# sml2004/CUDA-powered-mesh-handling-and-Iterative-solvers

Hardware: AMD Instinct MI355X
Metric: CG iterations/sec + DOFs/sec (assembly+solve), 10M P1-tet Poisson, 1/2/4/8 MI355X (higher is better)
Workload: dtype f64; 1 GPU; 10,110,954-tet P1 poisson Kuhn cube n=119, Jacobi-PCG fixed iterations; tets=10110954, nodes=1728000, dofs=1728000, nnz_blocks=25575838, parallelism=single GPU

## Files before the change

### cuda-powered-mesh-handling-and-iterative-solvers_amd/_capi.py

```python
from __future__ import annotations

import atexit
import ctypes
import functools
import inspect
import os
import threading

import torch

PKG_DIR = os.path.dirname(os.path.abspath(__file__))
LIB_PATH = os.environ.get("FEM355_LIB", os.path.join(PKG_DIR, "lib", "libfem355.so"))

FEM_OK, FEM_EBADTYPE, FEM_ESINGULAR, FEM_EHIP, FEM_ERCCL, FEM_EARG, FEM_ESTATE = range(7)
(PCG_RUNNING, PCG_CONVERGED, PCG_MAXITER, PCG_BREAKDOWN, PCG_ALPHA_NAN, PCG_BETA_NAN, PCG_SYNC_TIMEOUT,
 PCG_BAD_WINDOW) = range(8)
MODE_CG_STABLE, MODE_PCG, MODE_CG_CONSTRAINED = 0, 1, 2
TUNE_UPD1 = 1024
TUNE_U2_HOLD, TUNE_U2_SMALL = 2048, 4096
TUNE_MF_GATHER = 8192
TUNE_PK_GV = 16384
TUNE_PK_OFFDIAG = 32768
TUNE_PK_DESC = 65536
TUNE_DEFAULT = 1 | 2 | 4 | 8 | 128 | TUNE_UPD1 | TUNE_PK_OFFDIAG | TUNE_PK_DESC
KIND_ELASTIC, KIND_POISSON, KIND_MASS = 0, 1, 2
ISO_SUM, ISO_STACK, ISO_VOLUME, ISO_MASS = 0, 1, 2, 3
MASS_SELL, MASS_DIAG = 0, 1
MAT_SVK, MAT_NEO_HOOKEAN = 0, 1
MATERIALS = {"svk": MAT_SVK, "neo_hookean": MAT_NEO_HOOKEAN}
MAT_LINEAR = 2
EXPLICIT_MATERIALS = {"linear": MAT_LINEAR, **MATERIALS}
SURFACE_KINDS = {"plane": 0, "sphere": 1, "cylinder": 2}
XD_MAX_SURFACES = 8
SHELL_LOCAL, SHELL_POINTS, SHELL_GLOBAL = 0, 1, 2
LOAD_NONE, LOAD_UNIFORM, LOAD_NODAL, LOAD_ELEMENT = 0, 1, 2, 3
MODAL_OUT_GM, MODAL_OUT_NORMS, MODAL_OUT_LEN = 576, 1152, 1168

_P = ctypes.c_void_p
_I = ctypes.c_int
_L = ctypes.c_int64
_D = ctypes.c_double

SIGNATURES = {
    "fem_last_error": (ctypes.c_char_p, []),
    "fem_version": (_I, []),
    "fem_tet4_ke": (_I, [_P, _P, _L, _D, _D, _I, _P, _P, _P]),
    "fem_tet4_geom": (_I, [_P, _P, _L, _P, _P, _P, _P, _P]),
    "fem_iso_ke": (_I, [_P, _P, _L, _I, _D, _D, _P, _P, _I, _I, _P, _P]),
    "fem_iso_geom": (_I, [_P, _P, _L, _I, _P, _P, _P, _P, _P]),
    "fem_ke_sym_stride": (_I, [_I]),
    "fem_iso_ke_sym": (_I, [_P, _P, _L, _I, _D, _D, _P, _P, _I, _I, _P, _P]),
    "fem_assemble_from_ke_sym": (_I, [_P, _P, _I, _P, _P, _L, _P, _P, _P, _I, _I, _I, _P, _P]),
    "fem_assemble_from_ke_mass_sl": (_I, [_P, _P, _P, _I, _P, _P, _L, _P, _P, _P, _I, _I, _P, _P, _P]),
    "fem_iso_mass": (_I, [_P, _P, _L, _I, _D, _P, _P, _P, _I, _P, _P]),
    "fem_iso_mass_scalar": (_I, [_P, _P, _L, _I, _D, _P, _P, _P, _I, _P, _P]),
    "fem_pcg_scalars": (_I, [_P, ctypes.POINTER(_D)]),
    "fem_scan_work_len": (_L, [_L]),
    "fem_incidence_work_bytes": (_L, [_L, _L]),
    "fem_incidence": (_I, [_P, _L, _I, _L, _P, _P, _P, _P]),
    "fem_incidence_checked": (_I, [_P, _L, _I, _L, _P, _P, _P, _P, _P]),
    "fem_rcm_work_len": (_L, [_L]),
    "fem_rcm": (_I, [_P, _P, _L, _P, _P, _P, _P, _P]),
    "fem_graph_count": (_I, [_P, _I, _P, _P, _L, _P, _P, _P]),
    "fem_graph_fill": (_I, [_P, _I, _P, _P, _L, _P, _P, _P, _P]),
    "fem_graph_tmp_len": (_L, [_L]),
    "fem_graph_count2": (_I, [_P, _I, _P, _P, _L, _P, _P, _P, _P]),
    "fem_graph_fill2": (_I, [_P, _I, _P, _P, _L, _P, _P, _P, _P, _P]),
    "fem_graph_sell_fill": (_I, [_P, _I, _P, _P, _L, _P, _P, _P, _P, _P, _P, _P, _P, _P, _P]),
    "fem_graph_sell_fill_sl": (_I, [_P, _I, _P, _P, _L, _P, _P, _P, _P, _P, _P, _P, _I, _P, _P, _P, _P, _P]),
    "fem_scan_i32": (_I, [_P, _L, _P, _P, _P]),
    "fem_scan_i64": (_I, [_P, _L, _P, _P, _P]),
    "fem_sell_widths": (_I, [_P, _L, _P, _P]),
    "fem_graph_sizes": (_I, [_P, _P, _P, _L, _P, _P, _P, _P]),
    "fem_sell_fill": (_I, [_P, _P, _L, _P, _P, _P, _P]),
    "fem_sell_csr2sell": (_I, [_P, _L, _P, _P, _P]),
    "fem_assemble_from_ke": (_I, [_P, _P, _I, _I, _P, _P, _L, _P, _P, _P, _P, _P, _P]),
    "fem_assemble_from_ke_ex": (_I, [_P, _P, _I, _I, _P, _P, _L, _P, _P, _P, _P, _L, _L, _I, _P, _P]),
    "fem_assemble_from_ke_ex2": (_I, [_P, _P, _I, _I, _P, _P, _L, _P, _P, _P, _P, _L, _L, _I, _I, _P, _P]),
    "fem_assemble_tet4": (_I, [_P, _P, _D, _D, _I, _P, _P, _L, _P, _P, _P, _P, _P, _P, _P]),
    "fem_assemble_tet4_ex": (_I, [_P, _P, _D, _D, _I, _P, _P, _L, _P, _P, _P, _P, _I, _P, _P, _P]),
    "fem_assemble_tet4_ex2": (_I, [_P, _P, _D, _D, _I, _P, _P, _L, _P, _P, _P, _P, _I, _I, _P, _P, _P]),
    "fem_sell_to_csr_vals": (_I, [_P, _I, _P, _L, _P, _P, _P, _P]),
    "fem_jacobi": (_I, [_P, _I, _P, _P, _P, _P, _L, _P, _P, _P]),
    "fem_ebe_apply": (_I, [_P, _P, _I, _I, _P, _P, _L, _P, _P, _P]),
    "fem_ebe_diag": (_I, [_P, _P, _I, _I, _P, _P, _L, _I, _P, _P]),
    "fem_invert_diag": (_I, [_P, _L, _P, _P]),
    "fem_tet4_stress": (_I, [_P, _P, _L, _P, _D, _D, _P, _P, _P, _P]),
    "fem_iso_stress": (_I, [_P, _P, _L, _I, _P, _D, _D, _P, _P, _I, _I, _P, _P, _P]),
    "fem_voigt_to_tensor": (_I, [_P, _L, _P, _P]),
    "fem_von_mises": (_I, [_P, _L, _P, _P]),
    "fem_node_average": (_I, [_P, _I, _P, _P, _L, _P, _P]),
    "fem_face_forces": (_I, [_P, _P, _L, _I, _P, _P]),
    "fem_shared_face_sum": (_I, [_P, _P, _I, _L, _P, _P]),
    "fem_topo_create": (_I, [_P, _L, _I, _P, _I, _I, _L, _P, ctypes.POINTER(_P)]),
    "fem_topo_counts": (_I, [_P, ctypes.POINTER(_L), ctypes.POINTER(_L), ctypes.POINTER(_L)]),
    "fem_topo_pairs": (_I, [_P, _P]),
    "fem_topo_unique": (_I, [_P, _P]),
    "fem_topo_boundary": (_I, [_P, _P, _I, _P, _P, _P, _P, _P, ctypes.POINTER(_L)]),
    "fem_topo_destroy": (None, [_P]),
    "fem_sub_elements": (_I, [_P, _L, _I, _P, _I, _I, _P, _P]),
    "fem_element_face_normals": (_I, [_P, _P, _L, _I, _P, _P, _P, _P, _I, _D, _I, _I, _P, _P]),
    "fem_surface_normals": (_I, [_P, _P, _P, _L, _I, _I, _P, _P]),
    "fem_solid_ke": (_I, [_I, _P, _P, _L, _D, _D, _P, _P, _I, _I, _P, _P]),
    "fem_csr_pattern": (_I, [_P, _L, _I, _I, _L, _P, _P, _P, ctypes.POINTER(_L), _P]),
    "fem_csr_fill": (_I, [_P, _P, _L, _I, _I, _L, _P, _P, _P, _P]),
    "fem_spmv_csr": (_I, [_P, _P, _P, _P, _P, _L, _P]),
    "fem_pcg_csr": (_I, [_P, _P, _P, _L, _P, _P, _P, _P, _D, _I, _D, _I, ctypes.POINTER(_I), ctypes.POINTER(_I), _P,
                         _P]),
    "fem_vtk_read": (_I, [ctypes.c_char_p, ctypes.POINTER(_P)]),
    "fem_vtk_sizes": (_I, [_P, ctypes.POINTER(_L), ctypes.POINTER(_L), ctypes.POINTER(_L), ctypes.POINTER(_L)]),
    "fem_vtk_copy": (_I, [_P, _P, _P, _P]),
    "fem_vtk_free": (None, [_P]),
    "fem_spmv": (_I, [_L, _I, _P, _P, _P, _P, _P, _P]),
    "fem_sell_delta16": (_I, [_P, _L, _P, _P, _P, _P]),
    "fem_spmv16": (_I, [_L, _I, _P, _P, _P, _P, _P, _P]),
    "fem_pcg_set_cols16": (_I, [_P, _P]),
    "fem_pcg_set_tuning": (_I, [_P, _I]),
    "fem_stream_copy": (_I, [_P, _P, _L, _I, _P]),
    "fem_stream_read": (_I, [_P, _P, _L, _I, _P]),
    "fem_pcg_create": (_I, [_L, _I, _P, _P, _P, _P, _P, _P, _I, _D, _D, _P, _L, _P, ctypes.POINTER(_P)]),
    "fem_pcg_start": (_I, [_P]),
    "fem_pcg_iterate": (_I, [_P, _I]),
    "fem_pcg_poll": (_I, [_P, ctypes.POINTER(_I), ctypes.POINTER(_I), ctypes.POINTER(_D)]),
    "fem_pcg_sync_site": (_I, [_P, ctypes.POINTER(_I)]),
    "fem_pcg_debug_window": (_I, [_P, _I, _I, _I]),
    "fem_pcg_solve": (_I, [_P, _I, _I, ctypes.POINTER(_I), ctypes.POINTER(_I), ctypes.POINTER(_D)]),
    "fem_pcg_use_graph": (_I, [_P, _I]),
    "fem_pcg_set_schedule": (_I, [_P, _I]),
    "fem_pcg_set_entries": (_I, [_P, _L]),
    "fem_pcg_get_schedule": (_I, [_P]),
    "fem_pcg_uniform_slices": (_I, [_P, _L, _L, _P, _P, _P]),
    "fem_pcg_offdiag_slices": (_I, [_P, _P, _P, _P]),
    "fem_pcg_debug_offdiag": (_I, [_P, _P, _P]),
    "fem_pcg_desc_slices": (_I, [_P, _P, _P]),
    "fem_pcg_debug_desc": (_I, [_P, _P]),
    "fem_pcg_persist_build": (_I, [_P, ctypes.POINTER(_I), ctypes.POINTER(_I), ctypes.POINTER(_I)]),
    "fem_pcg_pipelined": (_I, [_P, ctypes.POINTER(_I)]),
    "fem_sell_sl_pattern": (_I, [_L, _P, _P, _I, _P, _P, _P, _P, _P]),
    "fem_assemble_tet4_sl": (_I, [_P, _P, _D, _D, _I, _P, _P, _L, _P, _P, _P, _P, _P, _I, _I, _P, _P, _P]),
    "fem_assemble_from_ke_sl": (_I, [_P, _P, _I, _P, _P, _L, _P, _P, _P, _I, _I, _P, _P]),
    "fem_jacobi_sl": (_I, [_P, _I, _P, _P, _P, _P, _P, _L, _P, _P, _P]),
    "fem_spmv_sl": (_I, [_L, _I, _P, _P, _P, _P, _P, _P, _P, _P]),
    "fem_sell_sl_unpair": (_I, [_L, _I, _P, _P, _P, _P, _P, _P, _P, _P]),
    "fem_pcg_set_layout": (_I, [_P, _P, _P, _P, _P, _P, _I]),
    "fem_pcg_persist_profile": (_I, [_P, _I, _P, ctypes.POINTER(_I)]),
    "fem_pcg_set_constraints": (_I, [_P, _I, _L, _P, _P, _L, _P, _P, _L, _P, _P, _P, _P, _P]),
    "fem_enforce_constraints": (_I, [_P, _P, _L, _I, _L, _P, _P, _L, _P, _P, _L, _P, _P, _P, _P, _P, _P]),
    "fem_pcg_finish": (_I, [_P]),
    "fem_pcg_profile": (_I, [_P, _I, _I, ctypes.POINTER(_D), ctypes.POINTER(_I)]),
    "fem_pcg_destroy": (None, [_P]),
    "fem_pcg_release_cache": (_I, []),
    "fem_release_scratch": (_I, []),
    "fem_pcg_set_rows": (_I, [_P, _I, _I, _P, _I]),
    "fem_pcg_comm_block": (_I, [_P, ctypes.POINTER(_P), ctypes.POINTER(_L)]),
    "fem_pcg_col_window": (_I, [_P, ctypes.POINTER(_L), ctypes.POINTER(_L)]),
    "fem_pcg_set_peers": (_I, [_P, _P, _P, _P]),
    "fem_pcg_dist_debug": (_I, [_P, _I, _P, _L]),
    "fem_stream_create_cu": (_I, [_I, _I, ctypes.POINTER(_P)]),
    "fem_stream_destroy": (_I, [_P]),
    "fem_pcg_set_prof": (_I, [_P, _P]),
    "fem_ipc_handle": (_I, [_P, ctypes.c_char_p]),
    "fem_ipc_open": (_I, [ctypes.c_char_p, ctypes.POINTER(_P)]),
    "fem_ipc_close": (_I, [_P]),
    "fem_sell_diag": (_I, [_P, _I, _P, _P, _L, _P, _P]),
    "fem_jacobi_from_diag": (_I, [_P, _L, _P, _P, _P]),
    "fem_mf_create": (_I, [_P, _P, _L, _L, _I, _D, _D, ctypes.POINTER(_L), _P, ctypes.POINTER(_P)]),
    "fem_mf_destroy": (_I, [_P]),
    "fem_mf_apply": (_I, [_P, _P, _P, _P]),
    "fem_mf_diag": (_I, [_P, _P, _P]),
    "fem_mf_info": (_I, [_P, ctypes.POINTER(_L)]),
    "fem_mf_order": (_I, [_P, _P, _P, _P, _P, _P]),
    "fem_pcg_set_operator_mf": (_I, [_P, _P]),
    "fem_comm_unique_id": (_I, [ctypes.c_char_p]),
    "fem_comm_init": (_I, [_I, _I, ctypes.c_char_p, ctypes.POINTER(_P)]),
    "fem_comm_destroy": (_I, [_P]),
    "fem_allreduce_sum": (_I, [_P, _P, _L, _P]),
    "fem_halo_sum": (_I, [_P, _P, _I, _P, _L, _P, _L, _P, _P]),
    "fem_halo_pack": (_I, [_P, _I, _P, _L, _P, _P]),
    "fem_halo_unpack": (_I, [_P, _I, _P, _L, _P, _P]),
    "fem_pcg_set_dist": (_I, [_P, _I, _P, _L, _P, _P, _P]),
    "fem_pcg_set_dist_variant": (_I, [_P, _I]),
    "fem_pcg_set_p2p": (_I, [_P, _I, _I, _P, _P, _P, _P]),
    "fem_pcg_p2p_buffers": (_I, [_P, ctypes.POINTER(_P), ctypes.POINTER(_P), ctypes.POINTER(_L)]),
    "fem_p2p_deliver": (_I, [_P, _I, _P]),
    "fem_pcg_dist_phase": (_I, [_P, _I]),
    "fem_pcg_dist_buffer": (_I, [_P, _I, ctypes.POINTER(_P), ctypes.POINTER(_L)]),
    "fem_group_allreduce": (_I, [_P, _I, _L, _P]),
    "fem_spmm": (_I, [_L, _I, _I, _P, _P, _P, _P, _P, _P, _P]),
    "fem_mpcg_create": (_I, [_L, _I, _I, _I, _P, _P, _P, _P, _P, _P, _P, _I, ctypes.POINTER(_D), _D, _P, _L, _P,
                             ctypes.POINTER(_P)]),
    "fem_mpcg_solve": (_I, [_P, _I, _I, ctypes.POINTER(_I), ctypes.POINTER(_I), ctypes.POINTER(_D)]),
    "fem_mpcg_scalars": (_I, [_P, ctypes.POINTER(_D)]),
    "fem_mpcg_destroy": (None, [_P]),
    "fem_coarse_restrict": (_I, [_L, _I, _I, _P, _P, _P, _P, _P, _P, _P]),
    "fem_coarse_apply": (_I, [_L, _I, _I, _P, _P, _P, _P, _P, _P, _P, _P, _P]),
    "fem_coarse_galerkin_count": (_I, [_L, _I, _P, _P, _P, _P, _P, _P]),
    "fem_coarse_galerkin": (_I, [_L, _I, _I, _P, _P, _P, _P, _P, _P, _P, _P, _P, _P, _P]),
    "fem_coarse_galerkin_sum": (_I, [_L, _I, _P, _P, _P, _P, _P, _P]),
    "fem_pcg2_create": (_I, [_L, _I, _P, _P, _P, _P, _P, _P, _P, _I, _P, _P, _P, _P, _P, _D, _P, _L, _P,
                             ctypes.POINTER(_P)]),
    "fem_pcg2_solve": (_I, [_P, _I, _I, ctypes.POINTER(_I), ctypes.POINTER(_I), ctypes.POINTER(_D)]),
    "fem_pcg2_scalars": (_I, [_P, ctypes.POINTER(_D)]),
    "fem_pcg2_destroy": (None, [_P]),
    "fem_refine_edge_slots": (_I, [_P, _L, _P, _L, _P, _P, _P]),
    "fem_refine_emit": (_I, [_P, _L, _L, _P, _P, _P, _P]),
    "fem_refine_nodes": (_I, [_P, _L, _P, _L, _P, _P, _P, _P]),
    "fem_mg_restrict": (_I, [_L, _L, _I, _P, _P, _P, _P, _P, _P]),
    "fem_mg_prolong": (_I, [_L, _L, _I, _P, _P, _P, _P, _P]),
    "fem_mg_create": (_I, [_I, _I, _P, _P, _P, _P, _P, _P, _P, _P, _P, _I, _P, _P, _L, _P, _P, ctypes.POINTER(_P)]),
    "fem_mg_apply": (_I, [_P, _P, _P]),
    "fem_mg_sweep": (_I, [_P, _I]),
    "fem_mg_solve": (_I, [_P, _P, _P, _D, _I, _I, _P, _L, ctypes.POINTER(_I), ctypes.POINTER(_I),
                          ctypes.POINTER(_D)]),
    "fem_mg_scalars": (_I, [_P, ctypes.POINTER(_D)]),
    "fem_mg_destroy": (None, [_P]),
    "fem_spmm_km": (_I, [_L, _I, _I, _P, _P, _P, _P, _P, _I, _P, _P, _P, _P]),
    "fem_modal_work_len": (_L, []),
    "fem_modal_gram": (_I, [_L, _I, _I, ctypes.POINTER(_P), _P, _P, _P]),
    "fem_modal_residual": (_I, [_L, _I, _P, _P, _P, _P, _P, _P, _P, _P]),
# ... 165 lines not shown
```

### cuda-powered-mesh-handling-and-iterative-solvers_amd/csrc/pcg.hip

```cpp
#include <rccl/rccl.h>
#include <stddef.h>

#include <atomic>
#include <mutex>
#include <vector>

#include "sell_pair.hpp"
#include "sell_pair3.hpp"
#include "matfree.hpp"

namespace fem {

template <typename T, bool NT>
__device__ __forceinline__ T ld(const T* p) {
    if constexpr (NT) return __builtin_nontemporal_load(p);
    else return *p;
}

struct VecPlain {
    const double* x;
    __device__ __forceinline__ double operator()(int64_t i) const { return x[i]; }
};
struct VecFusedP {
    const double* r;
// ... 1630 lines not shown
    for (int64_t i = (int64_t)blockIdx.x * blockDim.x + threadIdx.x; i < n; i += (int64_t)gridDim.x * blockDim.x)
        if (w[i] == 0.0) x[i] = 0.0;
}

}

using namespace fem;

struct fem_pcg {
    int64_t nrows, nslices, n;
    int bs;
    const int64_t* slice_ptr;
    const int32_t* cols;
    const double* vals;
    const double* b;
    double* x;
    const double* w;
    double* hist;
    int64_t hist_len;
    int mode;
    double tol, eps;
    hipStream_t stream;
    int fused;
    int deferred;
    int64_t launched;
    int64_t sell_ent;
    const int16_t* cols16;
    int has_con;
    int tune;
    int paired;
    double* pvals;
    int16_t* pcols16;
    int32_t* puoff;
    int16_t* pucol;
    int pext;
    const int32_t* pwin_ext;
    int pwin_G;
    Constraints con;
    double* r;
    double* p0;
    double* p1;
    double* q;
    RedBuf red;
    PcgState* st;
    PcgState* st_host;
    int grid_spmv, grid_vec;
    hipGraphExec_t graph;
    int graph_k;
    int max_iter;
    int dist;
    ncclComm_t comm;
    int64_t nI;
    const int32_t* imap;
    const int32_t* ipos;
    const uint8_t* own;
    double* hbuf;
    int cg1;
    double* cg1_s;
    double* cg1_u;
    double* cg1_send;
    double* cg1_recv;
    int p2p;
    int p2p_nranks;
    std::vector<int> peer_rank;
    std::vector<int64_t> peer_off, peer_cnt;
    int64_t p2p_total;
    const int32_t* p2p_csrc;
    const int32_t* p2p_ssrc;
    double* psend;
    double* precv;
    int c1f;
    int c1f_grid;
    int c1f_win_ok;
    int32_t* c1f_win;
    unsigned* c1f_flags;
    int persist_req;
    int persist_fit_only;
    int persist;
    int pk_grid;
    int pk_win_ok;
    int32_t* pk_win;
    double* pk_part;
    unsigned* pk_sync;
    int pk_ovf;
    double* pk_v;
    int pk_od;
    double* pk_ovals;
    int16_t* pk_oucol;
    int32_t* pk_kd;
    double* pk_diag;
    PkDesc* pk_desc;
    int pk_desc_on;
    int pk_coop;
    int pk_gv;
    double* gv_buf;
    int64_t gv_cap;
    int gv_init_pending;
    int64_t pk_epochs;
    hipEvent_t pev[2];
    int pd;
    int pd_rank, pd_nranks, pd_grid_req;
    int64_t pd_split[PK_MAX_RANKS + 1];
    char* pd_block;
    int64_t pd_block_bytes, pd_off_flag, pd_off_red, pd_off_rflag;
    int64_t pd_off_m1;
    char* pd_peer[PK_MAX_RANKS];
    int pd_peers_ok;
    int32_t* pd_pub;
    int pd_init_pending;
    unsigned long long* pd_prof;
    int upd1;
    int u2_grid;
    unsigned* u2_sync;
    fem_mf* mf;
    double* mf_sl;
    int64_t mf_sl_cap;
    int mf_nogather;
    int mf_qfuse;
};

#define FEM_NCCL(call)                                                                         \
    do {                                                                                       \
        ncclResult_t _r = (call);                                                              \
        if (_r != ncclSuccess) {                                                               \
            ::fem::set_error("%s:%d %s -> %s", __FILE__, __LINE__, #call, ncclGetErrorString(_r)); \
            return FEM_ERCCL;                                                                  \
        }                                                                                      \
    } while (0)

static const int16_t* pcols(const fem_pcg* s) { return s->bs == 1 ? s->pcols16 : s->cols16; }

template <class CI>
struct col_type {
    using type = CI;
};

template <class F>
static auto with_bs(int bs, F&& f) {
    return bs == 3 ? f(std::integral_constant<int, 3>{}) : f(std::integral_constant<int, 1>{});
}

template <class F>
static auto with_matrix(const fem_pcg* s, bool paired, F&& f) {
    return with_bs(s->bs, [&](auto B) {
        if (paired) return f(B, col_type<int16_t>{}, std::true_type{}, pcols(s), (const double*)s->pvals);
        if (s->cols16) return f(B, col_type<int16_t>{}, std::false_type{}, s->cols16, s->vals);
        return f(B, col_type<int32_t>{}, std::false_type{}, s->cols, s->vals);
    });
}
template <class F>
static auto with_matrix(const fem_pcg* s, F&& f) {
    return with_matrix(s, s->paired != 0, f);
}

static double* st_red(fem_pcg* s, int k) {
    return reinterpret_cast<double*>(reinterpret_cast<char*>(s->st) + offsetof(PcgState, red)) + k;
}

template <int BS>
__global__ void __launch_bounds__(MF_BLOCK) k_pcg_mf_dot(MfOp op, const double* __restrict__ p,
                                                         double* __restrict__ slots, PcgState* __restrict__ st,
                                                         RedBuf red) {
    __shared__ MfLds<BS> L;
    __shared__ double lds4[MF_BLOCK / 64];
    __shared__ int flag;
    if (blockIdx.x == 0 && threadIdx.x == 0) st->xupd = 0;
// ... 685 lines not shown
static const int64_t CON_SMALL = 8192;
static int launch_constraints(hipStream_t stream, double* x, double* r, const Constraints& c, const PcgState* st,
                              int always) {
    if (c.R + c.S <= CON_SMALL) {
        hipLaunchKernelGGL(k_constraints, dim3(1), dim3(256), 0, stream, x, r, c, st, always, 3);
        FEM_LAUNCHED();
        return FEM_OK;
    }
    auto phase = [&](int ph) {
        const int64_t m = ph == CON_SPC ? c.S : c.R;
        if (m == 0) return;
        const dim3 g(stream_grid(m, 256));
        if (ph == CON_GATHER) hipLaunchKernelGGL(k_con_phase<CON_GATHER>, g, dim3(256), 0, stream, x, r, c, st, always);
        if (ph == CON_SCATTER) hipLaunchKernelGGL(k_con_phase<CON_SCATTER>, g, dim3(256), 0, stream, x, r, c, st, always);
        if (ph == CON_SPC) hipLaunchKernelGGL(k_con_phase<CON_SPC>, g, dim3(256), 0, stream, x, r, c, st, always);
    };
    if (c.order == 0) {
        phase(CON_GATHER);
        phase(CON_SCATTER);
        phase(CON_SPC);
    } else {
        phase(CON_SPC);
        phase(CON_GATHER);
        phase(CON_SCATTER);
        if (c.G) hipLaunchKernelGGL(k_constraints, dim3(1), dim3(256), 0, stream, x, r, c, st, always, 2);
    }
    FEM_LAUNCHED();
    return FEM_OK;
}

static int launch_pupdate(fem_pcg* s) {
    if (s->fused) return FEM_OK;
    hipLaunchKernelGGL(k_pcg_pupdate, dim3(s->grid_vec), dim3(PCG_BLOCK), 0, s->stream, s->n, s->x, s->p0, s->r, s->w,
                       s->st);
    FEM_LAUNCHED();
    if (s->has_con) return launch_constraints(s->stream, s->x, nullptr, s->con, s->st, 0);
    return FEM_OK;
}

static int launch_update_finish(fem_pcg* s) {
    int rc;
    if ((rc = launch_update(s))) return rc;
    if (!s->dist) return FEM_OK;
    if ((rc = dist_exchange(s, 2))) return rc;
    hipLaunchKernelGGL(k_fin_rz, dim3(1), dim3(1), 0, s->stream, s->st, s->hist, s->hist_len);
    FEM_LAUNCHED();
    return FEM_OK;
}

static int launch_deferred(fem_pcg* s, int which) {
    const int par = (int)(s->launched & 1);
    const int rev = (s->tune & FEM_TUNE_REVERSE) ? par : 0;
    if (which == 0) {
        with_matrix(s, [&](auto B, auto ci, auto PAIR, auto* cols, const double* vals) {
            hipLaunchKernelGGL((k_pcg_d1<B(), typename decltype(ci)::type, PAIR()>), dim3(s->grid_spmv),
                               dim3(PCG_BLOCK), 0, s->stream, s->nslices, s->nrows, s->slice_ptr, cols, vals, s->p0, s->q,
                               s->st, par, rev, s->red.partials);
        });
    } else if (which == 1) {
        hipLaunchKernelGGL(k_pcg_d2, dim3(s->grid_vec), dim3(PCG_BLOCK), 0, s->stream, s->n, s->r, s->q, s->w, s->st,
                           par, s->red.partials, s->grid_spmv, s->red.partials + MAX_PARTIALS);
    } else {
        hipLaunchKernelGGL(k_pcg_d3, dim3(s->grid_vec), dim3(PCG_BLOCK), 0, s->stream, s->n, s->x, s->p0, s->r, s->w,
                           s->st, par, s->red.partials + MAX_PARTIALS, s->grid_vec, s->hist, s->hist_len);
        s->launched++;
    }
    FEM_LAUNCHED();
    return FEM_OK;
}

enum PkFamily { PKF_BS1, PKF_BS1_DIST, PKF_BS3, PKF_GV };

struct PkBuild {
    PkFamily fam;
    int slots;
    bool prof;
    bool gsc1;
    bool ovf;
    bool dist;
    bool od;
    const void* fn;
    size_t lds;
    bool desc;
};

template <int MAXS, bool PROF, bool GSC1, bool OVF = false, bool DIST = false, bool OD = false, bool DESC = false>
static PkBuild pk1_build() {
    return {DIST ? PKF_BS1_DIST : PKF_BS1, MAXS, PROF, GSC1, OVF, DIST, OD,
            (const void*)k_pcg_persist<MAXS, PROF, GSC1, OVF, DIST, OD, DESC>, PK_LDS, DESC};
}
template <bool OVF, bool DIST>
static PkBuild pk3_build() {
    return {PKF_BS3, P3_MAXS, false, true, OVF, DIST, false, (const void*)k_pcg_persist3<P3_MAXS, OVF, DIST>, P3_LDS};
}
template <int MAXS, bool DIST>
static PkBuild gv_build() {
    return {PKF_GV, MAXS, false, true, false, DIST, false, (const void*)k_pcg_persist_gv<MAXS, DIST>, GV_LDS};
}

constexpr int PK_MAXS_DIST = 4;

static const PkBuild PK_BUILDS[] = {
    pk1_build<1, false, true>(),
    pk1_build<2, false, true>(),
    pk1_build<4, false, true>(),
    pk1_build<PK_MAXS, false, true>(),
    pk1_build<PK_MAXS, false, false>(),
    pk1_build<PK_MAXS, true, true>(),
    pk1_build<PK_MAXS, true, false>(),
    pk1_build<PK_MAXS, false, true, true>(),
    pk1_build<PK_MAXS, false, false, true>(),
    pk1_build<1, false, true, false, false, true>(),
    pk1_build<2, false, true, false, false, true>(),
    pk1_build<4, false, true, false, false, true>(),
    pk1_build<PK_MAXS, false, true, false, false, true>(),
    pk1_build<PK_MAXS, false, false, false, false, true>(),
    pk1_build<PK_MAXS, true, true, false, false, true>(),
    pk1_build<PK_MAXS, true, false, false, false, true>(),
    pk1_build<PK_MAXS, false, true, true, false, true>(),
    pk1_build<PK_MAXS, false, false, true, false, true>(),
    pk1_build<1, false, true, false, false, true, true>(),
    pk1_build<2, false, true, false, false, true, true>(),
    pk1_build<4, false, true, false, false, true, true>(),
    pk1_build<PK_MAXS, false, true, false, false, true, true>(),
    pk1_build<PK_MAXS, true, true, false, false, true, true>(),
    pk1_build<1, false, true, false, true>(),
    pk1_build<2, false, true, false, true>(),
    pk1_build<PK_MAXS_DIST, false, true, false, true>(),
    pk1_build<PK_MAXS_DIST, true, true, false, true>(),
    pk1_build<PK_MAXS, false, true, false, true>(),
    pk1_build<PK_MAXS, true, true, false, true>(),
    pk3_build<false, false>(),
    pk3_build<true, false>(),
    pk3_build<false, true>(),
    gv_build<1, false>(),
    gv_build<2, false>(),
    gv_build<1, true>(),
    gv_build<2, true>(),
};

static const PkBuild* pk_find(PkFamily fam, int slots, bool prof, bool gsc1, bool ovf, bool dist, bool od,
                              bool desc = false) {
    for (const PkBuild& b : PK_BUILDS)
        if (b.fam == fam && b.slots == slots && b.prof == prof && b.gsc1 == gsc1 && b.ovf == ovf && b.dist == dist &&
            b.od == od && b.desc == desc)
            return &b;
    return nullptr;
}

static int pk_max_slots(PkFamily fam) {
    int m = 0;
    for (const PkBuild& b : PK_BUILDS)
        if (b.fam == fam && b.slots > m) m = b.slots;
    return m;
}

static int pk_pack(int64_t nslices, int G) {
    const int64_t maxL = (nslices + G - 1) / G;
    return (int)((maxL + PK_WAVES - 1) / PK_WAVES);
}

static int64_t pk_own_slices(const fem_pcg* s) {
    return s->pd ? s->pd_split[s->pd_rank + 1] - s->pd_split[s->pd_rank] : s->nslices;
}

struct PkPlan {
    const PkBuild* b;
    int pack;
};

static PkPlan persist_plan(const fem_pcg* s, bool prof, bool gv) {
    const int pk = pk_pack(pk_own_slices(s), s->pk_grid);
    const bool dist = s->pd != 0;
    if (gv) return {pk_find(PKF_GV, pk <= 1 ? 1 : 2, false, true, false, dist, false), pk};
    if (s->bs == 3) return {pk_find(PKF_BS3, P3_MAXS, false, true, !dist && s->pk_ovf, dist, false), pk};
    if (dist) {
        const int slots = !prof && pk <= 1 ? 1 : !prof && pk == 2 ? 2 : pk <= PK_MAXS_DIST ? PK_MAXS_DIST : PK_MAXS;
        return {pk_find(PKF_BS1_DIST, slots, prof, true, false, true, false), pk};
    }
    const int pack = (s->tune & FEM_TUNE_PK_PACK) ? pk : 0;
    const bool ovf = s->pk_ovf != 0, gsc1 = (s->tune & FEM_TUNE_PK_SC1) != 0;
    prof = prof && !ovf;
    const bool small = pack >= 1 && pack <= 4 && !(s->tune & FEM_TUNE_PK_WIDE) && !prof && !ovf && gsc1;
    const int slots = !small ? PK_MAXS : pack == 1 ? 1 : pack == 2 ? 2 : 4;
    const bool desc = s->pk_od && s->pk_desc_on && gsc1 && !ovf;
    return {pk_find(PKF_BS1, slots, prof, gsc1, ovf, false, s->pk_od != 0, desc), pack};
}
static PkPlan persist_plan(const fem_pcg* s, bool prof) { return persist_plan(s, prof, s->pk_gv && s->bs == 1); }

static int check_resident(const void* fn, int threads, size_t lds, int* nb) {
    FEM_HIP(hipFuncSetAttribute(fn, hipFuncAttributeMaxDynamicSharedMemorySize, (int)lds));
    FEM_HIP(hipOccupancyMaxActiveBlocksPerMultiprocessor(nb, fn, threads, lds));
    return FEM_OK;
}

static int family_resident(PkFamily fam, bool dist, int* res) {
    *res = 1;
    for (const PkBuild& b : PK_BUILDS) {
        if (b.fam != fam || b.dist != dist) continue;
        int nb = 0;
        const int rc = check_resident(b.fn, PK_T, b.lds, &nb);
        if (rc) return rc;
        if (nb < 1) {
            *res = 2;
            break;
        }
    }
    return FEM_OK;
}

static int launch_persist(fem_pcg* s, int k, unsigned long long* prof = nullptr);

static int launch_iterations(fem_pcg* s, int k) {
    if (s->dist && !s->comm) {
        set_error("distributed PCG without a communicator: drive it with fem_pcg_dist_phase");
        return FEM_EARG;
    }
    if (s->persist) return launch_persist(s, k);
    if (s->deferred && !s->dist) {
        for (int i = 0; i < k; ++i) {
            int rc;
            if ((rc = launch_deferred(s, 0)) || (rc = launch_deferred(s, 1)) || (rc = launch_deferred(s, 2))) return rc;
        }
        return FEM_OK;
    }
    if (s->dist && s->cg1) {
        for (int i = 0; i < k; ++i) {
            int rc;
            if ((rc = dist_phase(s, 4)) || (rc = dist_exchange(s, 4))) return rc;
            s->launched++;
        }
        return FEM_OK;
    }
    for (int i = 0; i < k; ++i) {
        int rc;
        if ((rc = launch_spmv_dot(s))) return rc;
        if (s->upd1) {
            if ((rc = launch_update2(s))) return rc;
        } else {
            if ((rc = launch_exchange_dot(s))) return rc;
            if ((rc = launch_update_finish(s))) return rc;
            if ((rc = launch_pupdate(s))) return rc;
        }
        s->launched++;
    }
    return FEM_OK;
}

template <class CI>
static int spmv_plain(const char* fn, int64_t nrows, int bs, const int64_t* slice_ptr, const CI* cols,
                      const double* vals, const double* x, double* y, fem_stream_t stream) {
    const int64_t ns = cdiv(nrows, 64);
    if (ns == 0) return FEM_OK;
    if (bs != 1 && bs != 3) {
        set_error("%s: block size %d unsupported", fn, bs);
        return FEM_EARG;
    }
    const int grid = grid_multiple_of_xcd(cdiv(ns, 4), 2048);
    with_bs(bs, [&](auto B) {
        hipLaunchKernelGGL((k_spmv<B(), SPMV_U, false, CI>), dim3(grid), dim3(256), 0, S(stream), ns, nrows, slice_ptr,
                           cols, vals, x, y);
    });
    FEM_LAUNCHED();
    return FEM_OK;
}

extern "C" {

// ... 76 lines not shown
    }
    Constraints c;
    const int rc = make_constraints("fem_pcg_set_constraints", s->n, s->stream, order, R, rbe2_slave, rbe2_master, S,
                                    spc_dof, spc_val, G, r3_ptr, r3_master, r3_wsum, r3_slave, r3_w, &c);
    if (rc != FEM_OK) return rc;
    if (s->con.tmp) (void)hipFree(s->con.tmp);
    s->con.tmp = nullptr;
    if (R > 0) FEM_HIP(hipMalloc(&c.tmp, sizeof(double) * (size_t)R));
    s->con = c;
    s->has_con = 1;
    return FEM_OK;
}

int fem_enforce_constraints(double* x, double* r, int64_t n, int order, int64_t R, const int64_t* rbe2_slave,
                            const int64_t* rbe2_master, int64_t S, const int64_t* spc_dof, const double* spc_val,
                            int64_t G, const int64_t* r3_ptr, const int64_t* r3_master, const double* r3_wsum,
                            const int64_t* r3_slave, const double* r3_w, fem_stream_t stream) {
    if (!x || n < 0) {
        set_error("fem_enforce_constraints: null x / negative n");
        return FEM_EARG;
    }
    const hipStream_t st = reinterpret_cast<hipStream_t>(stream);
    Constraints c;
    const int rc = make_constraints("fem_enforce_constraints", n, st, order, R, rbe2_slave, rbe2_master, S, spc_dof,
                                    spc_val, G, r3_ptr, r3_master, r3_wsum, r3_slave, r3_w, &c);
    if (rc != FEM_OK) return rc;
    if (R > 0) FEM_HIP(::fem::malloc_async((void**)&c.tmp, sizeof(double) * (size_t)R, st));
    const int lrc = launch_constraints(st, x, r, c, nullptr, 1);
    if (lrc != FEM_OK) return lrc;
    if (c.tmp) FEM_HIP(hipFreeAsync(c.tmp, st));
    return FEM_OK;
}

int fem_pcg_set_tuning(fem_pcg* s, int flags) {
    if (s->graph) {
        set_error("fem_pcg_set_tuning: drop the captured graph first");
        return FEM_EARG;
    }
    s->tune = flags;
    return FEM_OK;
}

int fem_pcg_set_cols16(fem_pcg* s, const int16_t* dcols) {
    if (s->graph) {
        set_error("fem_pcg_set_cols16: drop the captured graph first");
        return FEM_EARG;
    }
    s->cols16 = dcols;
    if (!dcols) s->paired = 0;
    return FEM_OK;
}

int fem_stream_copy(const double* src, double* dst, int64_t n, int grid, fem_stream_t stream) {
    if (grid <= 0) grid = 2048;
    hipLaunchKernelGGL(k_stream_copy, dim3(grid), dim3(256), 0, S(stream), (const double2*)src, (double2*)dst, n / 2);
    FEM_LAUNCHED();
    return FEM_OK;
}

int fem_stream_read(const double* src, double* out, int64_t n, int grid, fem_stream_t stream) {
    if (grid <= 0) grid = 4096;
    hipLaunchKernelGGL(k_stream_read, dim3(grid), dim3(256), 0, S(stream), (const double2*)src, n / 2, out);
    FEM_LAUNCHED();
    return FEM_OK;
}

int fem_pcg_create(int64_t nrows, int bs, const int64_t* slice_ptr, const int32_t* cols, const double* vals,
                   const double* b, double* x, const double* w, int mode, double tol, double eps, double* hist,
                   int64_t hist_len, fem_stream_t stream, fem_pcg** out) {
    if (bs != 1 && bs != 3) {
        set_error("fem_pcg_create: block size %d unsupported", bs);
        return FEM_EARG;
    }
    if (mode != FEM_MODE_CG_STABLE && mode != FEM_MODE_PCG && mode != FEM_MODE_CG_CONSTRAINED) {
        set_error("fem_pcg_create: unknown mode %d", mode);
        return FEM_EARG;
    }
    if (((uintptr_t)b | (uintptr_t)x | (uintptr_t)w) & 15) {
        set_error("fem_pcg_create: vectors must be 16-byte aligned");
        return FEM_EARG;
    }
    fem_pcg* s = new fem_pcg();
    s->tune = FEM_TUNE_REVERSE | FEM_TUNE_PAIR | FEM_TUNE_PK_SC1 | FEM_TUNE_PK_PACK | FEM_TUNE_PK_UNI | FEM_TUNE_UPD1 |
              FEM_TUNE_PK_OFFDIAG | FEM_TUNE_PK_DESC;
    s->nrows = nrows;
    s->bs = bs;
    s->nslices = cdiv(nrows, 64);
    s->n = nrows * bs;
    s->sell_ent = -1;
    s->slice_ptr = slice_ptr;
    s->cols = cols;
    s->vals = vals;
    s->b = b;
    s->x = x;
    s->w = w;
    s->hist = hist;
    s->hist_len = hist ? hist_len : 0;
    s->mode = mode;
    s->tol = tol;
    s->eps = eps;
    s->stream = S(stream);
    s->fused = 0;
    s->graph = nullptr;
    s->graph_k = 0;
    s->max_iter = 0x7fffffff;
    s->grid_spmv = grid_multiple_of_xcd(cdiv(s->nslices, 4), 2048);
    s->grid_vec = grid_multiple_of_xcd(cdiv(s->n / 2 + 1, PCG_BLOCK), 1024);
    size_t vec = sizeof(double) * (size_t)(s->n + 2);
    hipError_t e = hipSuccess;
    if (e == hipSuccess) e = pool_alloc((void**)&s->r, vec, s->stream, s->bs == 1);
    if (e == hipSuccess) e = pool_alloc((void**)&s->p0, vec, s->stream, s->bs == 1);
    if (e == hipSuccess) e = pool_alloc((void**)&s->p1, vec, s->stream, s->bs == 1);
    if (e == hipSuccess) e = pool_alloc((void**)&s->q, vec, s->stream, s->bs == 1);
    if (e == hipSuccess)
        e = pool_alloc((void**)&s->red.partials, sizeof(double) * RED_N * MAX_PARTIALS, s->stream, s->bs == 1);
    if (e == hipSuccess)
        e = pool_alloc((void**)&s->red.counters, sizeof(unsigned) * RED_N * RED_COUNTER_WORDS, s->stream, s->bs == 1);
    if (e == hipSuccess) e = hipMemsetAsync(s->red.counters, 0, sizeof(unsigned) * RED_N * RED_COUNTER_WORDS, s->stream);
    if (e == hipSuccess) e = pool_alloc((void**)&s->st, sizeof(PcgState), s->stream, s->bs == 1);
    if (e == hipSuccess) e = host_state_alloc((void**)&s->st_host, sizeof(PcgState));
    if (e != hipSuccess) {
        set_error("fem_pcg_create: allocation failed: %s", hipGetErrorString(e));
        fem_pcg_destroy(s);
        return FEM_EHIP;
    }
    *out = s;
    return FEM_OK;
}

int fem_pcg_set_operator_mf(fem_pcg* s, fem_mf* m) {
    if (!s || !m || mf_bs(m) != s->bs || mf_nodes(m) != s->nrows) {
        set_error("fem_pcg_set_operator_mf: the operator's block size / node count do not match the context");
        return FEM_EARG;
    }
    if (s->pd || s->has_con || s->graph || s->mode == FEM_MODE_CG_CONSTRAINED) {
        set_error("fem_pcg_set_operator_mf: contexts without constraints (CG_STABLE / PCG mode), the row-partitioned "
                  "schedule or a captured graph only");
        return FEM_EARG;
    }
    if (s->dist && !s->cg1) {
        set_error("fem_pcg_set_operator_mf: a distributed context runs the element-chunk operator in the "
                  "single-reduction variant only (fem_pcg_set_dist_variant(s, 1))");
        return FEM_EARG;
    }
    const int64_t need = (int64_t)mf_bs(m) * (int64_t)mf_nslots(m);
    if (need > s->mf_sl_cap) {
        if (s->mf_sl) FEM_HIP(hipFree(s->mf_sl));
        s->mf_sl = nullptr;
        s->mf_sl_cap = 0;
        FEM_HIP(hipMalloc(&s->mf_sl, sizeof(double) * (size_t)need));
        s->mf_sl_cap = need;
    }
    s->mf = m;
    {
        const char* e = getenv("FEM355_MF_NOGATHER");
        s->mf_nogather = e ? (atoi(e) != 0) : (int)(mf_nodes(m) >= MF_NOGATHER_MIN_NODES);
    }
    s->fused = s->deferred = s->persist_req = s->persist_fit_only = s->persist = 0;
    s->cols16 = nullptr;
    s->pext = 0;
    return FEM_OK;
}

int fem_pcg_set_entries(fem_pcg* s, int64_t entries) {
    if (entries < 0) {
        set_error("fem_pcg_set_entries: negative entry count %lld", (long long)entries);
        return FEM_EARG;
// ... 243 lines not shown
        for (int32_t k : h) c += k >= 0;
    }
    *od_slices = c;
    *bytes = c * 64 * (int64_t)sizeof(double);
    return FEM_OK;
}

static bool pk_runs_desc(const fem_pcg* s) {
    if (!s->persist || !s->pk_od || s->bs != 1 || s->pd || s->pk_gv) return false;
    const PkBuild* b = persist_plan(s, false, false).b;
    return b && b->desc;
}

int fem_pcg_desc_slices(fem_pcg* s, int64_t* desc_slices, int64_t* nslices) {
    *desc_slices = 0;
    *nslices = s->nslices;
    if (!pk_runs_desc(s) || s->nslices == 0) return FEM_OK;
    std::vector<PkDesc> h((size_t)s->nslices);
    FEM_HIP(hipMemcpyAsync(h.data(), s->pk_desc, sizeof(PkDesc) * h.size(), hipMemcpyDeviceToHost, s->stream));
    FEM_HIP(hipStreamSynchronize(s->stream));
    int64_t c = 0;
    for (const PkDesc& d : h) c += ((d.w[3] >> 8) & 0xffu) != (uint32_t)PKD_LANE;
    *desc_slices = c;
    return FEM_OK;
}

int fem_pcg_debug_desc(fem_pcg* s, uint32_t* records) {
    if (!pk_runs_desc(s)) {
        set_error("fem_pcg_debug_desc: the started context reads no descriptor records");
        return FEM_EARG;
    }
    FEM_HIP(hipMemcpyAsync(records, s->pk_desc, sizeof(PkDesc) * (size_t)s->nslices, hipMemcpyDeviceToHost, s->stream));
    FEM_HIP(hipStreamSynchronize(s->stream));
    return FEM_OK;
}

int fem_pcg_debug_offdiag(fem_pcg* s, const int32_t* rowptr, double* vals) {
    if (!s->persist || !s->pk_od || !s->cols16) {
        set_error("fem_pcg_debug_offdiag: the started context reads no diagonal-free stream");
        return FEM_EARG;
    }
    hipLaunchKernelGGL(k_sell_od_unpair, dim3(stream_grid(s->nslices * 64, 256)), dim3(256), 0, s->stream, s->nslices,
                       s->slice_ptr, s->cols16, s->puoff, s->pucol, s->pk_kd, s->pk_diag, rowptr, s->nrows,
                       s->pk_ovals, vals);
    FEM_LAUNCHED();
    FEM_HIP(hipStreamSynchronize(s->stream));
    return FEM_OK;
}

static int persist_setup(fem_pcg* s) {
    s->persist = 0;
    s->pk_od = 0;
    if (s->pd) return persist_setup_dist(s);
    if (!s->persist_req) return FEM_OK;
    if ((s->bs != 1 && s->bs != 3) || !s->paired || s->dist || s->mode == FEM_MODE_CG_CONSTRAINED || s->nslices == 0)
        return FEM_OK;
    int dev = 0, ncu = 0;
    FEM_HIP(hipGetDevice(&dev));
    FEM_HIP(hipDeviceGetAttribute(&ncu, hipDeviceAttributeMultiprocessorCount, dev));
    const int G = (ncu / NXCD) * NXCD;
    if (G < NXCD) return FEM_OK;
    const PkFamily fam = s->bs == 3 ? PKF_BS3 : PKF_BS1;
    const bool ovf = s->nslices > (int64_t)G * PK_WAVES * pk_max_slots(fam);
    if (ovf && (!(s->tune & FEM_TUNE_PK_PACK) || s->persist_fit_only)) return FEM_OK;
    static std::mutex occ_mu;
    static int occ_cache[2][64] = {};
    int occ;
    {
        std::lock_guard<std::mutex> lk(occ_mu);
        int& slot = occ_cache[s->bs == 3][dev & 63];
        if (slot == 0) {
            int res = 0;
            const int rc = family_resident(fam, false, &res);
            if (rc) return rc;
            slot = res;
        }
        occ = slot;
    }
    if (occ != 1) return FEM_OK;
    if (s->pk_grid != G) {
        pool_free(s->pk_win, s->stream);
        pool_free(s->pk_part, s->stream);
        pool_free(s->pk_sync, s->stream);
        s->pk_win = nullptr;
        s->pk_part = nullptr;
        s->pk_sync = nullptr;
        FEM_HIP(pool_alloc((void**)&s->pk_win, sizeof(int32_t) * 2 * G, s->stream, s->bs == 1));
        FEM_HIP(pool_alloc((void**)&s->pk_part, sizeof(double) * 4 * G, s->stream, s->bs == 1));
        FEM_HIP(pool_alloc((void**)&s->pk_sync, sizeof(unsigned) * pk_sync_words(G), s->stream, s->bs == 1));
        s->pk_grid = G;
        s->pk_win_ok = 0;
    }
    if (!s->pk_win_ok && s->pwin_ext && s->pwin_G == G) {
        FEM_HIP(hipMemcpyAsync(s->pk_win, s->pwin_ext, sizeof(int32_t) * 2 * G, hipMemcpyDeviceToDevice, s->stream));
        s->pk_win_ok = 1;
    }
    if (!s->pk_win_ok) {
        hipLaunchKernelGGL(k_pk_window_init, dim3(cdiv(G, 256)), dim3(256), 0, s->stream, G, G, s->pk_win);
        FEM_LAUNCHED();
        hipLaunchKernelGGL(k_pk_window, dim3(stream_grid(s->nslices * 64, 256)), dim3(256), 0, s->stream, s->nslices,
                           s->nrows, s->slice_ptr, s->cols16, G, s->pk_win, s->pk_win + G);
        FEM_LAUNCHED();
        s->pk_win_ok = 1;
    }
    if (ovf && !s->pk_v) FEM_HIP(pool_alloc((void**)&s->pk_v, sizeof(double) * (size_t)s->n, s->stream, s->bs == 1));
    s->pk_ovf = ovf ? 1 : 0;
    s->persist = 1;
    s->pk_gv = 0;
    if ((s->tune & FEM_TUNE_PK_GV) && (s->tune & FEM_TUNE_PK_SC1) && s->bs == 1 && !ovf && s->mode == FEM_MODE_PCG) {
        if (pk_pack(s->nslices, G) <= pk_max_slots(PKF_GV)) {
            static std::mutex gv_mu;
            static int gv_ok[64] = {};
            std::lock_guard<std::mutex> lk(gv_mu);
            int& slot = gv_ok[dev & 63];
            if (slot == 0) {
                int res = 0;
                const int rc = family_resident(PKF_GV, false, &res);
                if (rc) return rc;
                slot = res;
            }
            s->pk_gv = slot == 1;
        }
    }
    return offdiag_build(s);
}

static int persist_setup_dist(fem_pcg* s) {
    if ((s->bs != 1 && s->bs != 3) || !s->paired || s->dist || s->mode == FEM_MODE_CG_CONSTRAINED) {
        set_error("distributed persistent PCG: needs bs = 1 or 3, 16-bit columns with the paired copy, no element "
                  "partition, no constraints");
        return FEM_EARG;
    }
    if (!s->pd_peers_ok) {
        set_error("distributed persistent PCG: fem_pcg_set_peers first");
        return FEM_EARG;
    }
    const int G = s->pk_grid;
    const int64_t nloc = pk_own_slices(s);
    if ((nloc + G - 1) / G > (int64_t)PK_WAVES * pk_max_slots(s->bs == 3 ? PKF_BS3 : PKF_BS1_DIST)) {
        set_error("distributed persistent PCG: %lld slices on this rank exceed the register capacity of %d workgroups",
                  (long long)nloc, G);
        return FEM_EARG;
    }
    s->pk_ovf = 0;
    s->pk_gv = 0;
    for (int prof = 0; prof < (s->bs == 3 ? 1 : 2); ++prof) {
        const PkBuild* b = persist_plan(s, prof != 0, false).b;
        int nb = 0;
        const int rc = b ? check_resident(b->fn, PK_T, b->lds, &nb) : FEM_OK;
        if (rc) return rc;
        if (nb < 1) {
            set_error("distributed persistent PCG: kernel does not fit one workgroup per CU");
            return FEM_EARG;
        }
    }
    s->persist = 1;
    if (s->pd_off_m1 > 0 && s->mode == FEM_MODE_PCG && pk_pack(nloc, G) <= pk_max_slots(PKF_GV)) {
        int res = 0;
        const int rc = family_resident(PKF_GV, true, &res);
        if (rc) return rc;
        s->pk_gv = res == 1;
    }
    return FEM_OK;
}

static int persist_reset_sync(fem_pcg* s) {
    FEM_HIP(hipMemsetAsync(s->pk_sync, 0, sizeof(unsigned) * pk_sync_words(s->pk_grid), s->stream));
    FEM_HIP(hipMemsetAsync(&s->st->pk_epoch, 0, sizeof(unsigned), s->stream));
    s->pk_epochs = 0;
    return FEM_OK;
}

static PkArgs pk_args(const fem_pcg* s, const PkPlan& plan, int k, unsigned long long* prof) {
    const bool bs3 = s->bs == 3;
    const bool uni = (s->tune & FEM_TUNE_PK_UNI) && s->puoff;
    const bool od = plan.b->od;
    PkArgs a;
    a.nslices = pk_own_slices(s);
    a.nrows = s->nrows;
    a.slice_ptr = s->slice_ptr;
    a.cols = pcols(s);
    a.vals = od ? s->pk_ovals : s->pvals;
    a.uoff = uni && !bs3 ? s->puoff : nullptr;
    a.ucol = bs3 ? nullptr : od ? s->pk_oucol : uni ? s->pucol : nullptr;
    a.x = s->x;
    a.r = s->r;
    a.p = s->p0;
    a.s = s->p1;
    a.u = s->pd ? reinterpret_cast<double*>(s->pd_block) : s->q;
    a.w = s->w;
    a.win = s->pk_win;
    a.part = s->pk_part;
    a.sync = s->pk_sync;
    a.st = s->st;
    a.hist = s->hist;
    a.hist_len = s->hist_len;
    a.kmax = k;
    a.rev = (s->tune & FEM_TUNE_REVERSE) ? 1 : 0;
    a.prof = prof;
    a.v = s->pk_ovf ? s->pk_v : nullptr;
    a.pack = plan.pack;
    a.sbase = s->pd ? s->pd_split[s->pd_rank] : 0;
    a.rank = s->pd ? s->pd_rank : 0;
    a.nranks = s->pd ? s->pd_nranks : 1;
    for (int q = 0; q < PK_MAX_RANKS; ++q) a.peer[q] = s->pd && q < s->pd_nranks ? s->pd_peer[q] : nullptr;
    a.off_flag = s->pd ? s->pd_off_flag : 0;
    a.off_red = s->pd ? s->pd_off_red : 0;
    a.off_rflag = s->pd ? s->pd_off_rflag : 0;
    a.pub = s->pd ? s->pd_pub : nullptr;
    a.b = s->b;
    a.init = s->pd ? s->pd_init_pending : 0;
    a.diag = od ? s->pk_diag : nullptr;
    a.vals_full = s->pvals;
    a.ucol_full = uni ? s->pucol : nullptr;
    a.desc = plan.b->desc ? s->pk_desc : nullptr;
    return a;
}

static GvArgs gv_args(const fem_pcg* s) {
    const int64_t n = s->n;
    GvArgs g;
    g.u = s->gv_buf;
    g.w = s->gv_buf + n;
    g.q = s->gv_buf + 2 * n;
    g.z = s->gv_buf + 3 * n;
    g.m[0] = s->pd ? reinterpret_cast<double*>(s->pd_block) : s->gv_buf + 4 * n;
    g.m[1] = s->pd ? reinterpret_cast<double*>(s->pd_block + s->pd_off_m1) : s->gv_buf + 5 * n;
    g.moff[0] = 0;
    g.moff[1] = s->pd ? s->pd_off_m1 : 0;
    g.init = s->pd ? 0 : s->gv_init_pending;
    return g;
}

static int launch_persist(fem_pcg* s, int k, unsigned long long* prof) {
    const int G = s->pk_grid;
    if (s->pk_epochs + k + 1 > (int64_t(1) << 24)) {
        if (s->pd) {
            set_error("distributed persistent PCG: 2^24 iterations since fem_pcg_start; restart the solve");
            return FEM_EARG;
        }
        const int rc = persist_reset_sync(s);
        if (rc) return rc;
    }
    s->pk_epochs += k + 1;
    const bool gv = s->pk_gv && s->bs == 1;
    if (prof && (gv || (s->bs == 3 && !s->pd))) {
        set_error("persistent PCG: no instrumented (PROF) build %s", gv ? "of the pipelined iteration" : "for bs = 3");
        return FEM_EARG;
    }
    if (s->pd && !prof && !gv) prof = s->pd_prof;
    if (s->bs == 3) prof = nullptr;
    const PkPlan plan = persist_plan(s, prof != nullptr);
    if (!plan.b) {
        set_error("persistent PCG: no build for this context (%d slices per wave)", plan.pack);
        return FEM_ESTATE;
    }
    PkArgs a = pk_args(s, plan, k, prof);
    s->pd_init_pending = 0;
    GvArgs g;
    void* args[] = {&a, &g};
    if (gv) {
        g = gv_args(s);
        s->gv_init_pending = 0;
        s->pk_epochs += 2;
    }
    if (s->pk_coop || (s->tune & FEM_TUNE_PK_COOP))
        FEM_HIP(hipLaunchCooperativeKernel(plan.b->fn, dim3(G), dim3(PK_T), args, plan.b->lds, s->stream));
    else
        FEM_HIP(hipLaunchKernel(plan.b->fn, dim3(G), dim3(PK_T), args, plan.b->lds, s->stream));
    FEM_LAUNCHED();
    s->launched += k;
    return FEM_OK;
}

int fem_pcg_pipelined(fem_pcg* s, int* on) {
    *on = (s && s->persist && s->pk_gv) ? 1 : 0;
    return FEM_OK;
}

int fem_pcg_persist_build(fem_pcg* s, int* slots, int* overflow, int* pack) {
    *slots = 0;
    *overflow = 0;
    *pack = 0;
    if (!s->persist || s->pk_grid <= 0) return FEM_OK;
    const PkPlan plan = persist_plan(s, false, false);
    *slots = plan.b ? plan.b->slots : 0;
    *overflow = s->pk_ovf;
    *pack = plan.pack;
    return FEM_OK;
}

__global__ void __launch_bounds__(256) k_sell_sl_pattern(int64_t nslices, int64_t nrows,
                                                         const int64_t* __restrict__ slice_ptr,
                                                         const int16_t* __restrict__ cin, int16_t* __restrict__ pout,
                                                         int16_t* __restrict__ ucol, int32_t* __restrict__ uoff, int G,
                                                         int* __restrict__ win, int2* __restrict__ span) {
    __shared__ int cand_all[4][SU_MAXW];
    const int64_t s = ((int64_t)blockIdx.x * blockDim.x + threadIdx.x) >> 6;
    if (s >= nslices) return;
    const int l = threadIdx.x & 63;
    const int64_t p0 = slice_ptr[s];
    sl_pattern_slice(s, l, nslices, nrows, slice_ptr, [&](int k) { return (int)cin[p0 + 64 * k + l]; }, pout, ucol,
                     uoff, G, win, cand_all[(threadIdx.x >> 6) & 3], span);
}

static PcgState state_view(const fem_pcg* s) {
    PcgState h = *s->st_host;
    if (s->deferred && !s->dist && !s->persist) {
        const PcgState::Bank& b = h.bank[s->launched & 1];
        h.iter = b.iter;
        h.status = b.status;
        h.halt = b.halt;
        h.stop_iter = b.stop_iter;
        h.rz = b.rz;
        h.rz_new = b.rz_new;
        h.pq = b.pq;
        h.alpha = b.alpha;
        h.beta = b.beta;
    }
    return h;
}

static int refresh_pairing(fem_pcg* s) {
    const bool want = (s->bs == 1 || s->bs == 3) && s->cols16 && (s->tune & FEM_TUNE_PAIR) && !s->fused;
    s->paired = 0;
    if (s->pext) {
        if (!want) {
            set_error("PCG: a solver-layout matrix needs the paired schedules (FEM_TUNE_PAIR, 16-bit columns, not fused)");
            return FEM_EARG;
        }
        s->paired = 1;
        return FEM_OK;
    }
    if (!want || s->nslices == 0) return FEM_OK;
    int64_t ent = s->sell_ent;
    if (ent < 0) {
        FEM_HIP(hipMemcpyAsync(&ent, s->slice_ptr + s->nslices, sizeof(int64_t), hipMemcpyDeviceToHost, s->stream));
        FEM_HIP(hipStreamSynchronize(s->stream));
    }
    if (s->bs == 3) {
        if (!s->pvals) FEM_HIP(pool_alloc((void**)&s->pvals, sizeof(double) * 9 * (size_t)ent, s->stream, s->bs == 1));
        s->pcols16 = nullptr;
        hipLaunchKernelGGL(k_sell3_to_a, dim3(stream_grid(s->nslices * 64, 256)), dim3(256), 0, s->stream, s->nslices,
                           s->slice_ptr, s->vals, s->pvals);
        FEM_LAUNCHED();
        s->paired = 1;
        return FEM_OK;
    }
    if (!s->pvals) {
        FEM_HIP(pool_alloc((void**)&s->pvals, sizeof(double) * (size_t)ent, s->stream, s->bs == 1));
        FEM_HIP(pool_alloc((void**)&s->pcols16, sizeof(int16_t) * (size_t)ent, s->stream, s->bs == 1));
    }
    s->paired = 1;
    if ((s->tune & FEM_TUNE_PK_UNI) && 2 * (ent / 64) + 2 < (int64_t)INT32_MAX) {
        if (!s->puoff) {
            FEM_HIP(pool_alloc((void**)&s->puoff, sizeof(int32_t) * (size_t)s->nslices, s->stream, true));
            FEM_HIP(pool_alloc((void**)&s->pucol, sizeof(int16_t) * (size_t)(2 * (ent / 64) + 2), s->stream, true));
        }
        hipLaunchKernelGGL(k_sell_uniform, dim3((unsigned)cdiv(s->nslices, 4)), dim3(256), 0, s->stream, s->nslices,
                           s->nrows, s->slice_ptr, s->vals, s->cols16, s->pvals, s->pcols16, s->pucol, s->puoff, 1);
        FEM_LAUNCHED();
        return FEM_OK;
    }
    hipLaunchKernelGGL(k_sell_pair, dim3(stream_grid(s->nslices * 64, 256)), dim3(256), 0, s->stream, s->nslices,
                       s->slice_ptr, s->vals, s->cols16, s->pvals, s->pcols16);
    FEM_LAUNCHED();
    return FEM_OK;
}

static int gv_ensure(fem_pcg* s) {
    const int64_t need = 6 * s->n;
    if (need > s->gv_cap) {
        pool_free(s->gv_buf, s->stream);
        s->gv_buf = nullptr;
        s->gv_cap = 0;
        FEM_HIP(pool_alloc((void**)&s->gv_buf, sizeof(double) * (size_t)need, s->stream, true));
        s->gv_cap = need;
    }
    FEM_HIP(hipMemsetAsync(s->gv_buf, 0, sizeof(double) * (size_t)need, s->stream));
    return FEM_OK;
}

int fem_pcg_start(fem_pcg* s) {
    if (s->mf && s->dist && !s->cg1) {
        set_error("fem_pcg_start: a distributed element-chunk context needs the single-reduction variant "
                  "(fem_pcg_set_dist_variant(s, 1))");
        return FEM_EARG;
    }
    {
        int prc = refresh_pairing(s);
        if (!prc) prc = persist_setup(s);
        if (!prc) prc = c1f_setup(s);
        if (!prc) prc = u2_setup(s);
        if (prc) return prc;
    }
    PcgState h{};
    h.tol = s->tol;
    h.eps = s->eps;
    h.mode = s->mode;
    h.max_iter = s->max_iter;
    h.x_done = 1;
    h.dist = s->dist;
    *s->st_host = h;
    FEM_HIP(hipMemcpyAsync(s->st, s->st_host, sizeof(PcgState), hipMemcpyHostToDevice, s->stream));
    int rc;
    if (s->dist) {
        if (!s->comm) return FEM_OK;
        if (s->cg1) {
            if ((rc = dist_phase(s, 10)) || (rc = dist_exchange(s, 10)) || (rc = dist_phase(s, 20)) ||
                (rc = dist_exchange(s, 20)))
                return rc;
            return FEM_OK;
        }
        if ((rc = dist_phase(s, 10)) || (rc = dist_exchange(s, 10)) || (rc = dist_phase(s, 11)) ||
            (rc = dist_exchange(s, 11)) || (rc = dist_phase(s, 12)))
            return rc;
        return FEM_OK;
    }
    if (s->mode == FEM_MODE_CG_STABLE) {
        hipLaunchKernelGGL(k_zero_fixed, dim3(stream_grid(s->n, 256)), dim3(256), 0, s->stream, s->n, s->x, s->w);
        FEM_LAUNCHED();
    }
    if (s->pd) {
        if (!s->persist) {
            set_error("distributed persistent PCG: setup failed");
            return FEM_EARG;
        }
        FEM_HIP(hipMemsetAsync(s->pk_sync, 0, sizeof(unsigned) * pk_sync_words(s->pk_grid), s->stream));
        FEM_HIP(hipMemsetAsync(s->pd_block, 0, (size_t)s->pd_block_bytes, s->stream));
        FEM_HIP(hipMemsetAsync(&s->st->pk_epoch, 0, sizeof(unsigned), s->stream));
        s->pk_epochs = 0;
        s->pd_init_pending = 1;
        s->launched = 0;
        if (s->pk_gv && (rc = gv_ensure(s))) return rc;
        return FEM_OK;
    }
    if ((rc = start_spmv(s, true))) return rc;
    if (s->persist) {
        const int zrc = persist_reset_sync(s);
        if (zrc) return zrc;
        if (s->pk_gv) {
            if ((rc = gv_ensure(s))) return rc;
            s->gv_init_pending = 1;
        }
        hipLaunchKernelGGL(k_cg1_init, dim3(s->grid_vec), dim3(PCG_BLOCK), 0, s->stream, s->n, s->bs, s->b, s->r,
                           s->q, s->w, s->p0, s->p1, s->q, (const uint8_t*)nullptr, s->st, s->red);
        FEM_LAUNCHED();
        s->launched = 0;
        return FEM_OK;
    }
    hipLaunchKernelGGL(k_pcg_init, dim3(s->grid_vec), dim3(PCG_BLOCK), 0, s->stream, s->n, s->b, s->r, s->q, s->w, s->p0,
                       s->p1, s->fused, s->st, s->red, (const uint8_t*)nullptr, s->bs);
    FEM_LAUNCHED();
    if (s->has_con) {
        const int rc = launch_constraints(s->stream, s->x, nullptr, s->con, s->st, 1);
        if (rc != FEM_OK) return rc;
    }
    s->launched = 0;
    if (s->deferred) {
        hipLaunchKernelGGL(k_bank_init, dim3(1), dim3(1), 0, s->stream, s->st);
        FEM_LAUNCHED();
    }
    return FEM_OK;
}

int fem_pcg_dist_phase(fem_pcg* s, int phase) {
    if (!s->dist) {
        set_error("fem_pcg_dist_phase: context is not in distributed mode");
        return FEM_EARG;
    }
    return dist_phase(s, phase);
}

int fem_pcg_dist_buffer(fem_pcg* s, int phase, double** ptr, int64_t* n) {
    dist_buffer(s, phase, ptr, n);
    return FEM_OK;
}

int fem_comm_unique_id(char* out128) {
    ncclUniqueId id;
    FEM_NCCL(ncclGetUniqueId(&id));
    memcpy(out128, id.internal, sizeof(id.internal));
    return FEM_OK;
}

int fem_comm_init(int nranks, int rank, const char* id128, void** comm) {
    ncclUniqueId id;
    memcpy(id.internal, id128, sizeof(id.internal));
    ncclComm_t c;
    FEM_NCCL(ncclCommInitRank(&c, nranks, id, rank));
    *comm = c;
    return FEM_OK;
}

int fem_comm_destroy(void* comm) {
    if (comm) FEM_NCCL(ncclCommDestroy((ncclComm_t)comm));
    return FEM_OK;
}

int fem_allreduce_sum(void* comm, double* buf, int64_t n, fem_stream_t stream) {
    FEM_NCCL(ncclAllReduce(buf, buf, (size_t)n, ncclFloat64, ncclSum, (ncclComm_t)comm, S(stream)));
    return FEM_OK;
}

int fem_halo_pack(const double* v, int bs, const int32_t* imap, int64_t nI, double* buf, fem_stream_t stream) {
    if (nI <= 0) return FEM_OK;
    hipLaunchKernelGGL(k_halo_pack, dim3(stream_grid(nI * bs, 256)), dim3(256), 0, S(stream), v, bs, imap, nI, buf,
                       (const PcgState*)nullptr, 0);
    FEM_LAUNCHED();
    return FEM_OK;
}
// ... 355 lines not shown
        const bool dfr = s->deferred && !s->dist;
        if (s->upd1) {
            (void)hipEventRecord(evs[4 * si + 0], s->stream);
            rc = launch_spmv_dot(s);
            (void)hipEventRecord(evs[4 * si + 1], s->stream);
            if (!rc) rc = launch_update2(s);
            (void)hipEventRecord(evs[4 * si + 2], s->stream);
            (void)hipEventRecord(evs[4 * si + 3], s->stream);
            s->launched++;
            ++si;
            continue;
        }
        (void)hipEventRecord(evs[4 * si + 0], s->stream);
        rc = dfr ? launch_deferred(s, 0) : launch_spmv_dot(s);
        (void)hipEventRecord(evs[4 * si + 1], s->stream);
        if (!rc && !dfr) rc = launch_exchange_dot(s);
        if (!rc) rc = dfr ? launch_deferred(s, 1) : launch_update_finish(s);
        (void)hipEventRecord(evs[4 * si + 2], s->stream);
        if (!rc) rc = dfr ? launch_deferred(s, 2) : launch_pupdate(s);
        (void)hipEventRecord(evs[4 * si + 3], s->stream);
        ++si;
    }
    FEM_HIP(hipStreamSynchronize(s->stream));
    for (int i = 0; i < si; ++i) {
        float t;
        for (int j = 0; j < 3; ++j) {
            const bool c1 = s->dist && s->cg1;
            (void)hipEventElapsedTime(&t, evs[4 * i + (c1 && j == 2 ? 3 : j)], evs[4 * i + (c1 && j == 2 ? 0 : j + 1)]);
            acc[j] += t;
        }
    }
    for (auto& e : evs) (void)hipEventDestroy(e);
    for (int j = 0; j < 3; ++j) {
        if (ms) ms[j] = acc[j];
        if (n) n[j] = si;
    }
    return rc;
}

int fem_pcg_set_rows(fem_pcg* s, int nranks, int rank, const int64_t* slice_split, int grid) {
    if (nranks < 1 || nranks > PK_MAX_RANKS || rank < 0 || rank >= nranks || !slice_split) {
        set_error("fem_pcg_set_rows: nranks %d (1..%d), rank %d", nranks, PK_MAX_RANKS, rank);
        return FEM_EARG;
    }
    if ((s->bs != 1 && s->bs != 3) || s->dist || s->mode == FEM_MODE_CG_CONSTRAINED || s->pd) {
        set_error("fem_pcg_set_rows: bs = 1 or 3, not element-partitioned, not constrained, once per context");
        return FEM_EARG;
    }
    if (slice_split[0] != 0 || slice_split[nranks] != s->nslices) {
        set_error("fem_pcg_set_rows: the split must cover slices [0, %lld)", (long long)s->nslices);
        return FEM_EARG;
    }
    for (int q = 0; q < nranks; ++q)
        if (slice_split[q + 1] <= slice_split[q]) {
            set_error("fem_pcg_set_rows: rank %d owns no slice", q);
            return FEM_EARG;
        }
    int dev = 0, ncu = 0;
    FEM_HIP(hipGetDevice(&dev));
    FEM_HIP(hipDeviceGetAttribute(&ncu, hipDeviceAttributeMultiprocessorCount, dev));
    const int G = grid > 0 ? grid : (ncu / NXCD) * NXCD;
    if (G < NXCD || G % NXCD || G > ncu) {
        set_error("fem_pcg_set_rows: grid %d must be a multiple of %d within %d CUs", G, NXCD, ncu);
        return FEM_EARG;
    }
    s->pd_rank = rank;
    s->pd_nranks = nranks;
    for (int q = 0; q <= nranks; ++q) s->pd_split[q] = slice_split[q];
    const int64_t line = sizeof(unsigned) * PK_LINE;
    const int64_t vreg = (int64_t)cdiv(sizeof(double) * (s->n + 2), 256) * 256;
    s->pd_off_m1 = ((s->tune & FEM_TUNE_PK_GV) && s->bs == 1) ? vreg : 0;
    s->pd_off_flag = vreg + s->pd_off_m1;
    s->pd_off_red = s->pd_off_flag + (int64_t)nranks * G * line;
    s->pd_off_rflag = s->pd_off_red + 256;
    s->pd_block_bytes = s->pd_off_rflag + PK_MAX_RANKS * NXCD * line;
    if (s->tune & FEM_TUNE_DIST_FINE)
        FEM_HIP(hipExtMallocWithFlags((void**)&s->pd_block, (size_t)s->pd_block_bytes, hipDeviceMallocFinegrained));
    else
        FEM_HIP(hipMalloc((void**)&s->pd_block, (size_t)s->pd_block_bytes));
    FEM_HIP(hipMemsetAsync(s->pd_block, 0, (size_t)s->pd_block_bytes, s->stream));
    pool_free(s->pk_win, s->stream);
    pool_free(s->pk_part, s->stream);
    pool_free(s->pk_sync, s->stream);
    FEM_HIP(pool_alloc((void**)&s->pk_win, sizeof(int32_t) * (2 * G + 2), s->stream, true));
    FEM_HIP(pool_alloc((void**)&s->pk_part, sizeof(double) * 4 * G, s->stream, true));
    FEM_HIP(pool_alloc((void**)&s->pk_sync, sizeof(unsigned) * pk_sync_words(G), s->stream, true));
    s->pk_grid = G;
    std::vector<int32_t> lohi(2 * (size_t)G + 2);
    for (int i = 0; i < G; ++i) {
        lohi[i] = nranks * G;
        lohi[G + i] = -1;
    }
    lohi[2 * G] = 0x7fffffff;
    lohi[2 * G + 1] = -1;
    FEM_HIP(hipMemcpyAsync(s->pk_win, lohi.data(), sizeof(int32_t) * lohi.size(), hipMemcpyHostToDevice, s->stream));
    PkSplit sp{};
    for (int q = 0; q <= nranks; ++q) sp.b[q] = slice_split[q];
    const int64_t nloc = slice_split[rank + 1] - slice_split[rank];
    hipLaunchKernelGGL(k_pk_window_dist, dim3(stream_grid(nloc * 64, 256)), dim3(256), 0, s->stream, slice_split[rank],
                       nloc, s->nrows, s->slice_ptr, s->cols, G, sp, nranks, s->pk_win, s->pk_win + G,
                       s->pk_win + 2 * G);
    FEM_LAUNCHED();
    FEM_HIP(hipStreamSynchronize(s->stream));
    s->pk_win_ok = 1;
    s->pd = 1;
    s->pd_peers_ok = 0;
    s->persist_req = 1;
    s->deferred = 1;
    s->fused = 0;
    return FEM_OK;
}

int fem_pcg_comm_block(fem_pcg* s, void** base, int64_t* bytes) {
    if (!s->pd) {
        set_error("fem_pcg_comm_block: fem_pcg_set_rows first");
        return FEM_EARG;
    }
    if (base) *base = s->pd_block;
    if (bytes) *bytes = s->pd_block_bytes;
    return FEM_OK;
}

int fem_pcg_col_window(fem_pcg* s, int64_t* lo, int64_t* hi) {
    if (!s->pd) {
        set_error("fem_pcg_col_window: fem_pcg_set_rows first");
        return FEM_EARG;
    }
    int32_t w[2];
    FEM_HIP(hipMemcpyAsync(w, s->pk_win + 2 * s->pk_grid, sizeof w, hipMemcpyDeviceToHost, s->stream));
    FEM_HIP(hipStreamSynchronize(s->stream));
    *lo = w[0];
    *hi = w[1];
    return FEM_OK;
}

int fem_pcg_set_peers(fem_pcg* s, void* const* bases, const int64_t* need_lo, const int64_t* need_hi) {
    if (!s->pd) {
        set_error("fem_pcg_set_peers: fem_pcg_set_rows first");
        return FEM_EARG;
    }
    const int N = s->pd_nranks, G = s->pk_grid, r = s->pd_rank;
    for (int q = 0; q < N; ++q) {
        s->pd_peer[q] = q == r ? s->pd_block : (char*)bases[q];
        if (!s->pd_peer[q]) {
            set_error("fem_pcg_set_peers: no comm block for rank %d", q);
            return FEM_EARG;
        }
    }
    const int64_t S0 = s->pd_split[r], nloc = s->pd_split[r + 1] - S0;
    auto owner = [&](int64_t row) {
        const int64_t sl = row >> 6;
        int q = 0;
        while (q + 1 < N && s->pd_split[q + 1] <= sl) ++q;
        const int64_t S = s->pd_split[q + 1] - s->pd_split[q], tl = sl - s->pd_split[q];
        const int64_t L = ((tl + 1) * G - 1) / S;
        return (int64_t)q * G + (L < G ? L : G - 1);
    };
    std::vector<int32_t> pub((size_t)G * N * 2, -1);
    for (int q = 0; q < N && !(s->tune & FEM_TUNE_DIST_DROP); ++q) {
        if (q == r || need_hi[q] < need_lo[q]) continue;
        const int64_t glo = owner(need_lo[q]), ghi = owner(need_hi[q]);
        for (int L = 0; L < G; ++L) {
            const int64_t Lg = (int64_t)r * G + L;
            if (Lg < glo || Lg > ghi) continue;
            const int64_t rlo = (S0 + (int64_t)L * nloc / G) * 64;
            const int64_t rhi = std::min<int64_t>((S0 + (int64_t)(L + 1) * nloc / G) * 64, s->nrows);
            const int64_t lo = std::max<int64_t>(rlo, need_lo[q]), hi = std::min<int64_t>(rhi, need_hi[q] + 1);
            pub[((size_t)L * N + q) * 2] = (int32_t)std::max<int64_t>(lo, 0);
            pub[((size_t)L * N + q) * 2 + 1] = (int32_t)std::max<int64_t>(hi, std::max<int64_t>(lo, 0));
// ... 44 lines not shown
        return FEM_EARG;
    }
    std::vector<uint32_t> mask((size_t)(ncu + 31) / 32, 0u);
    for (int cu = 0; cu < ncu; ++cu)
        if (cu % nparts == part) mask[(size_t)cu / 32] |= 1u << (cu % 32);
    hipStream_t st = nullptr;
    FEM_HIP(hipExtStreamCreateWithCUMask(&st, (uint32_t)mask.size(), mask.data()));
    *stream = st;
    return FEM_OK;
}

int fem_stream_destroy(void* stream) {
    FEM_HIP(hipStreamDestroy(reinterpret_cast<hipStream_t>(stream)));
    return FEM_OK;
}

int fem_pcg_set_prof(fem_pcg* s, unsigned long long* dev_buf) {
    if (!s->pd) {
        set_error("fem_pcg_set_prof: distributed persistent contexts only (single GPU: fem_pcg_persist_profile)");
        return FEM_EARG;
    }
    s->pd_prof = dev_buf;
    return FEM_OK;
}

int fem_ipc_handle(void* ptr, char* out64) {
    hipIpcMemHandle_t h;
    FEM_HIP(hipIpcGetMemHandle(&h, ptr));
    static_assert(sizeof(h) <= 64, "IPC handle size");
    memset(out64, 0, 64);
    memcpy(out64, &h, sizeof h);
    return FEM_OK;
}

int fem_ipc_open(const char* h64, void** ptr) {
    hipIpcMemHandle_t h;
    memcpy(&h, h64, sizeof h);
    FEM_HIP(hipIpcOpenMemHandle(ptr, h, hipIpcMemLazyEnablePeerAccess));
    return FEM_OK;
}

int fem_ipc_close(void* ptr) {
    FEM_HIP(hipIpcCloseMemHandle(ptr));
    return FEM_OK;
}

void fem_pcg_destroy(fem_pcg* s) {
    if (!s) return;
    if (s->pev[0]) (void)hipEventDestroy(s->pev[0]);
    if (s->pd_block) (void)hipFree(s->pd_block);
    if (s->pd_pub) (void)hipFree(s->pd_pub);
    if (s->pev[1]) (void)hipEventDestroy(s->pev[1]);
    if (s->graph) (void)hipGraphExecDestroy(s->graph);
    pool_free(s->r, s->stream);
    pool_free(s->p0, s->stream);
    pool_free(s->p1, s->stream);
    pool_free(s->q, s->stream);
    pool_free(s->red.partials, s->stream);
    pool_free(s->red.counters, s->stream);
    if (s->hbuf) (void)hipFree(s->hbuf);
    if (s->cg1_s) (void)hipFree(s->cg1_s);
    if (s->cg1_u) (void)hipFree(s->cg1_u);
    if (s->cg1_send) (void)hipFree(s->cg1_send);
    if (s->cg1_recv) (void)hipFree(s->cg1_recv);
    if (s->psend) (void)hipFree(s->psend);
    if (s->precv) (void)hipFree(s->precv);
    if (s->c1f_win) (void)hipFree(s->c1f_win);
    if (s->c1f_flags) (void)hipFree(s->c1f_flags);
    if (s->con.tmp) (void)hipFree(s->con.tmp);
    if (s->mf_sl) (void)hipFree(s->mf_sl);
    if (s->pext) {
        s->pvals = nullptr;
        s->pcols16 = nullptr;
        s->puoff = nullptr;
        s->pucol = nullptr;
    }
    pool_free(s->pvals, s->stream);
    pool_free(s->pcols16, s->stream);
    pool_free(s->puoff, s->stream);
    pool_free(s->pucol, s->stream);
    pool_free(s->pk_win, s->stream);
    pool_free(s->pk_part, s->stream);
    pool_free(s->pk_sync, s->stream);
    pool_free(s->pk_v, s->stream);
    pool_free(s->pk_ovals, s->stream);
    pool_free(s->pk_oucol, s->stream);
    pool_free(s->pk_desc, s->stream);
    pool_free(s->pk_kd, s->stream);
    pool_free(s->pk_diag, s->stream);
    pool_free(s->gv_buf, s->stream);
    pool_free(s->u2_sync, s->stream);
    pool_free(s->st, s->stream);
    host_state_free(s->st_host, s->stream);
    delete s;
}

}
```

### cuda-powered-mesh-handling-and-iterative-solvers_amd/csrc/pcg_persist.hpp

```cpp
#pragma once
#include "sell_pair.hpp"

namespace fem {

constexpr int PK_MAXS = 7;
constexpr int PK_U = 2;
template <int MAXS, bool PROF>
constexpr int pk_u() { return MAXS <= 1 ? 8 : (MAXS <= 4 && !PROF) ? 4 : PK_U; }
template <int MAXS, bool PROF>
constexpr int pk_u_rec() { return MAXS <= 1 ? 4 : pk_u<MAXS, PROF>(); }
constexpr int PK_LINE = 32;
enum { PK_GRP = 0, PK_TOP = 8 * PK_LINE, PK_GEN = 9 * PK_LINE, PK_TMO = 17 * PK_LINE, PK_UFLAG = 18 * PK_LINE };
constexpr uint64_t PK_WAIT_TICKS = 200000000ull;
constexpr uint64_t PK_RANK_WAIT_TICKS = 500000000ull;
__device__ __forceinline__ uint64_t pk_now() { return __builtin_amdgcn_s_memrealtime(); }
__device__ __forceinline__ bool pk_expired(uint64_t t0, uint64_t ticks) { return pk_now() - t0 > ticks; }
constexpr int PK_NPROF = 8;
constexpr size_t PK_LDS_HEAD = 256;
constexpr int PK_VL = 5;
constexpr size_t PK_LDS = PK_LDS_HEAD + sizeof(double) * (2 * PK_MAXS + PK_VL) * PK_WAVES * 64;
static_assert(PK_LDS <= 160 * 1024, "persistent PCG: LDS over the 160 KB of a CU");

template <class T>
__device__ __forceinline__ T* pk_launder(T* p) {
    __attribute__((address_space(1))) T* q = (__attribute__((address_space(1))) T*)p;
    asm volatile("" : "+s"(q));
    return (T*)q;
}

__device__ __forceinline__ unsigned pk_ld(const unsigned* p) {
    return __hip_atomic_load(p, __ATOMIC_RELAXED, __HIP_MEMORY_SCOPE_AGENT);
}
__device__ __forceinline__ void pk_st(unsigned* p, unsigned v) {
    __hip_atomic_store(p, v, __ATOMIC_RELAXED, __HIP_MEMORY_SCOPE_AGENT);
}

__device__ __forceinline__ bool pk_wait_ge(const unsigned* p, unsigned target, unsigned* tmo) {
    const uint64_t t0 = pk_now();
    for (unsigned spins = 0;; ++spins) {
        if (pk_ld(p) >= target) return true;
        if ((spins & 63) == 63 && pk_ld(tmo)) return false;
        if ((spins & 63) == 63 && pk_expired(t0, PK_WAIT_TICKS)) {
            pk_st(tmo, 1u + 16u * (target / NXCD));
            return false;
        }
        __builtin_amdgcn_s_sleep(2);
    }
}

__device__ __forceinline__ double pk_sum(const double* part, int n) {
    const int lane = threadIdx.x & 63;
    double v = 0.0;
    for (int i = lane; i < n; i += 64) v += __hip_atomic_load(part + i, __ATOMIC_RELAXED, __HIP_MEMORY_SCOPE_AGENT);
    return wave_sum(v);
}

__device__ __forceinline__ bool pk_barrier(unsigned* sy, int grp, unsigned nper, unsigned e, int* lds_ok,
                                           const double* pd, const double* pg, int G, double* out,
                                           bool entry_sync = true) {
    if (entry_sync) __syncthreads();
    if (threadIdx.x < 64) {
        int okv = 0;
        if (threadIdx.x == 0) {
            asm volatile("s_waitcnt vmcnt(0)" ::: "memory");
            unsigned* tmo = sy + PK_TMO;
            bool ok;
            const unsigned old = __hip_atomic_fetch_add(sy + PK_GRP + grp * PK_LINE, 1u, __ATOMIC_RELAXED,
                                                        __HIP_MEMORY_SCOPE_AGENT);
            if (old == e * nper - 1)
                for (int r = 0; r < NXCD; ++r)
                    __hip_atomic_fetch_add(sy + PK_GEN + r * PK_LINE, 1u, __ATOMIC_RELAXED, __HIP_MEMORY_SCOPE_AGENT);
            ok = pk_wait_ge(sy + PK_GEN + grp * PK_LINE, e * NXCD, tmo);
            okv = ok ? 1 : 0;
        }
        okv = __builtin_amdgcn_readfirstlane(okv);
        if (okv && pd) {
            const int lane = threadIdx.x & 63;
            double vd = 0.0, vg = 0.0;
            if (pg) {
#pragma unroll 4
                for (int i = lane; i < G; i += 64) {
                    const double a = __hip_atomic_load(pd + i, __ATOMIC_RELAXED, __HIP_MEMORY_SCOPE_AGENT);
                    const double b = __hip_atomic_load(pg + i, __ATOMIC_RELAXED, __HIP_MEMORY_SCOPE_AGENT);
                    vd += a;
                    vg += b;
                }
            } else {
#pragma unroll 4
                for (int i = lane; i < G; i += 64) vd += __hip_atomic_load(pd + i, __ATOMIC_RELAXED, __HIP_MEMORY_SCOPE_AGENT);
            }
            const double d = wave_sum(vd);
            const double g = pg ? wave_sum(vg) : 0.0;
            if (threadIdx.x == 0) {
                out[0] = d;
                out[1] = g;
            }
        }
        if (threadIdx.x == 0) *lds_ok = okv;
    }
    __syncthreads();
    return *lds_ok != 0;
}

__device__ __forceinline__ double pk_block_sum(double v, double* lds16) {
    v = wave_sum(v);
    const int w = threadIdx.x >> 6;
    if ((threadIdx.x & 63) == 0) lds16[w] = v;
    __syncthreads();
    double t = 0.0;
    if (threadIdx.x == 0) {
#pragma unroll
        for (int i = 0; i < PK_WAVES; ++i) t += lds16[i];
    }
    return t;
}

constexpr int PK_MAX_RANKS = 8;

struct PkArgs {
    int64_t nslices, nrows;
    const int64_t* slice_ptr;
    const int16_t* cols;
    const double* vals;
    const int32_t* uoff;
    const int16_t* ucol;
    double* x;
    double* r;
    double* p;
    double* s;
    double* u;
    const double* w;
    const int32_t* win;
    double* part;
    unsigned* sync;
    PcgState* st;
    double* hist;
    int64_t hist_len;
    int kmax;
    int rev;
    int pack;
    double* v;
    unsigned long long* prof;
    int64_t sbase;
    int rank, nranks;
    char* peer[PK_MAX_RANKS];
    int64_t off_flag, off_red, off_rflag;
    const int32_t* pub;
    const double* b;
    int init;
    const double* diag;
    const double* vals_full;
    const int16_t* ucol_full;
    const PkDesc* desc;
};

__device__ __forceinline__ double pk_mul_rn(double a, double b) {
    double m = a * b;
    asm("" : "+v"(m));
    return m;
}

__device__ __forceinline__ bool pk_barrier_dist(const PkArgs& a, unsigned* sy, int grp, unsigned nper, unsigned e,
                                                int* lds_ok, const double* pd, const double* pg, int G, double* out,
                                                bool entry_sync = true) {
    if (entry_sync) __syncthreads();
    if (threadIdx.x < 64) {
        const int lane = threadIdx.x;
        unsigned* tmo = sy + PK_TMO;
        int last = 0;
        if (lane == 0) {
            asm volatile("s_waitcnt vmcnt(0)" ::: "memory");
            const unsigned old = __hip_atomic_fetch_add(sy + PK_GRP + grp * PK_LINE, 1u, __ATOMIC_RELAXED,
                                                        __HIP_MEMORY_SCOPE_AGENT);
            if (old == e * nper - 1) {
                const unsigned old2 = __hip_atomic_fetch_add(sy + PK_GEN, 1u, __ATOMIC_RELAXED, __HIP_MEMORY_SCOPE_AGENT);
                last = old2 == e * NXCD - 1;
            }
        }
        last = __builtin_amdgcn_readfirstlane(last);
        const int bank = (int)(e & 1u);
        if (last) {
            double vd = 0.0, vg = 0.0;
#pragma unroll 4
            for (int i = lane; i < G; i += 64) {
                vd += __hip_atomic_load(pd + i, __ATOMIC_RELAXED, __HIP_MEMORY_SCOPE_AGENT);
                if (pg) vg += __hip_atomic_load(pg + i, __ATOMIC_RELAXED, __HIP_MEMORY_SCOPE_AGENT);
            }
            const double d = wave_sum(vd), g = wave_sum(vg);
            if (lane < a.nranks) {
                double* red = reinterpret_cast<double*>(a.peer[lane] + a.off_red) + (bank * PK_MAX_RANKS + a.rank) * 2;
                __hip_atomic_store(red, d, __ATOMIC_RELAXED, __HIP_MEMORY_SCOPE_SYSTEM);
                __hip_atomic_store(red + 1, g, __ATOMIC_RELAXED, __HIP_MEMORY_SCOPE_SYSTEM);
            }
            __builtin_amdgcn_fence(__ATOMIC_RELEASE, "");
            asm volatile("s_waitcnt vmcnt(0)" ::: "memory");
            if (lane < a.nranks * NXCD)
                __hip_atomic_store(reinterpret_cast<unsigned*>(a.peer[lane / NXCD] + a.off_rflag) +
                                       (a.rank * NXCD + lane % NXCD) * PK_LINE,
                                   e, __ATOMIC_RELAXED, __HIP_MEMORY_SCOPE_SYSTEM);
        }
        const unsigned* rf = reinterpret_cast<const unsigned*>(a.peer[a.rank] + a.off_rflag);
        int okv = 1;
        bool done = lane >= a.nranks;
        const uint64_t t0 = pk_now();
        for (unsigned spins = 0; !__all(done); ++spins) {
            if (!done)
                done = __hip_atomic_load(rf + (lane * NXCD + grp) * PK_LINE, __ATOMIC_RELAXED,
                                         __HIP_MEMORY_SCOPE_SYSTEM) >= e;
            if ((spins & 63) == 63 && pk_ld(tmo)) {
                okv = 0;
                break;
            }
            if ((spins & 63) == 63 && pk_expired(t0, PK_RANK_WAIT_TICKS)) {
                pk_st(tmo, 3u + 16u * e);
                okv = 0;
                break;
            }
            __builtin_amdgcn_s_sleep(1);
        }
        if (okv) {
            const double* red = reinterpret_cast<const double*>(a.peer[a.rank] + a.off_red) + bank * PK_MAX_RANKS * 2;
            double d = 0.0, g = 0.0;
            for (int q = 0; q < a.nranks; ++q) {
                d += __hip_atomic_load(red + 2 * q, __ATOMIC_RELAXED, __HIP_MEMORY_SCOPE_SYSTEM);
                g += __hip_atomic_load(red + 2 * q + 1, __ATOMIC_RELAXED, __HIP_MEMORY_SCOPE_SYSTEM);
            }
            if (lane == 0) {
                out[0] = d;
                out[1] = g;
            }
        }
        if (lane == 0) *lds_ok = okv;
    }
    __syncthreads();
    return *lds_ok != 0;
}

__device__ __forceinline__ void pk_publish_row(const PkArgs& a, int L, unsigned pubmask, unsigned row, double v) {
    for (int q = 0; q < a.nranks; ++q) {
        if (!(pubmask & (1u << q))) continue;
        const int32_t* pr = a.pub + (L * a.nranks + q) * 2;
        if ((int)row >= pr[0] && (int)row < pr[1])
            __hip_atomic_store(reinterpret_cast<double*>(a.peer[q]) + row, v, __ATOMIC_RELAXED,
                               __HIP_MEMORY_SCOPE_SYSTEM);
    }
}

__device__ __forceinline__ void pk_publish_flag(const PkArgs& a, int Lg, unsigned pubmask, unsigned e) {
    for (int q = 0; q < a.nranks; ++q)
        if (pubmask & (1u << q))
            __hip_atomic_store(reinterpret_cast<unsigned*>(a.peer[q] + a.off_flag) + Lg * PK_LINE, e, __ATOMIC_RELAXED,
                               __HIP_MEMORY_SCOPE_SYSTEM);
}


#define PK_ON(j) ((j) < nreg && lane < nrows - (s0 + (j)) * 64)

template <int MAXS, bool PROF, bool GSC1, bool OVF = false, bool DIST = false, bool OD = false, bool DESC = false>
__global__ void __launch_bounds__(PK_T) k_pcg_persist(PkArgs a) {
    static_assert(!DIST || (GSC1 && !OVF), "distributed persistent PCG: sc1 gathers, no overflow build");
    static_assert(!(DIST && OD), "distributed persistent PCG: no diagonal-free stream");
    static_assert(!DESC || (OD && GSC1 && !OVF), "descriptor records: the diagonal-free sc1 builds without overflow");
    unsigned long long pacc[PROF ? PK_NPROF : 1] = {};
    unsigned long long pt = 0, wspmv = 0;
    if constexpr (PROF) pt = __builtin_amdgcn_s_memtime();
#define PK_MARK(i)                                                         \
    __builtin_amdgcn_sched_barrier(0);                                     \
    if constexpr (PROF) {                                                  \
        const unsigned long long now = __builtin_amdgcn_s_memtime();       \
        pacc[i] += now - pt;                                               \
        pt = now;                                                          \
    }
    extern __shared__ __attribute__((aligned(16))) double pk_lds_raw[];
    double* lds16 = pk_lds_raw;
    int& lds_ok = *reinterpret_cast<int*>(pk_lds_raw + PK_WAVES);
    double* lds_dg = pk_lds_raw + PK_WAVES + 2;
    double* pk_lds = pk_lds_raw + PK_LDS_HEAD / sizeof(double);
    const int G = gridDim.x;
    const unsigned nper = (unsigned)(G / NXCD);
    const int L = (blockIdx.x % NXCD) * (G / NXCD) + blockIdx.x / NXCD;
    const int grp = L / (int)nper;
    const int lane = threadIdx.x & 63;
    const int wv = __builtin_amdgcn_readfirstlane(threadIdx.x >> 6);
    int s0, nsl;
    if (a.pack) {
        const int m = a.pack;
        const int sL0 = (int)((int64_t)L * a.nslices / G);
        const int nL = (int)((int64_t)(L + 1) * a.nslices / G) - sL0;
        const int lo = wv * m < nL ? wv * m : nL;
        s0 = sL0 + lo + (DIST ? (int)a.sbase : 0);
        nsl = nL - lo < m ? nL - lo : m;
    } else {
        const int64_t W = (int64_t)G * PK_WAVES;
        const int64_t gw = (int64_t)L * PK_WAVES + wv;
        s0 = (int)(gw * a.nslices / W);
        nsl = (int)((gw + 1) * a.nslices / W) - s0;
    }
    const int nreg = (OVF && nsl > MAXS) ? MAXS : nsl;
    const int nov = nsl - nreg;
    const int nrows = (int)a.nrows;
    const unsigned rb = (unsigned)s0 * 64u + (unsigned)lane;
    double* xl = pk_lds + wv * MAXS * 64 + lane;
    double* wl = pk_lds + PK_WAVES * MAXS * 64 + wv * MAXS * 64 + lane;
    double* vl = pk_lds + 2 * PK_WAVES * MAXS * 64 + wv * PK_VL * 64 + lane;
    unsigned* sy = a.sync;
    PcgState* st = a.st;
    unsigned* uf = DIST ? reinterpret_cast<unsigned*>(a.peer[a.rank] + a.off_flag) : sy + PK_UFLAG;
    const int Lg = DIST ? a.rank * G + L : L;
    const int olo = DIST ? (int)(a.sbase * 64) : 0;
    const int ohi = DIST ? (int)((a.sbase + a.nslices) * 64 < a.nrows ? (a.sbase + a.nslices) * 64 : a.nrows) : 0;
    unsigned pubmask = 0;
    bool ghost = false;
    if constexpr (DIST) {
        for (int q = 0; q < a.nranks; ++q)
            if (q != a.rank && a.pub[(L * a.nranks + q) * 2] >= 0) pubmask |= 1u << q;
        ghost = a.win[L] < a.rank * G || a.win[G + L] >= (a.rank + 1) * G;
    }

    const bool cg = st->mode != FEM_MODE_PCG;
    const double tol = st->tol, eps = st->eps;
    const int max_iter = st->max_iter;
    int it = st->iter, halt = st->halt, status = st->status, stop_iter = st->stop_iter;
    double rz = st->rz, alpha_prev = st->alpha, beta = st->beta, pq = st->pq, rz_new = st->rz_new;
    double g = st->red[1];
    unsigned ebase = st->pk_epoch;
    unsigned elast = ebase;

    double rr[MAXS], pp[MAXS], ss[MAXS], vv[MAXS];
    double uo[OD ? 1 : MAXS];
    double dg[OD ? MAXS : 1];
#define PK_UO(j) (OD ? pk_mul_rn(wl[(j) * 64], rr[j]) : uo[OD ? 0 : (j)])
#pragma unroll
    for (int j = 0; j < MAXS; ++j) {
        const unsigned row = rb + 64u * j;
        const bool on = PK_ON(j);
        rr[j] = on ? a.r[row] : 0.0;
        pp[j] = on ? a.p[row] : 0.0;
        ss[j] = on ? a.s[row] : 0.0;
        vv[j] = 0.0;
        xl[j * 64] = on ? a.x[row] : 0.0;
        if (j < PK_VL) vl[j * 64] = 0.0;
        const double wj = on ? a.w[row] : 0.0;
        wl[j * 64] = wj;
        if constexpr (OD) dg[j] = on ? a.diag[row] : 0.0;
        else uo[j] = wj * rr[j];
    }
    const int nflags = (DIST ? a.nranks : 1) * G;
    const int wraw0 = a.win[L], wraw1 = a.win[G + L];
    const int wlo = max(wraw0, 0), whi = min(wraw1, nflags - 1);
    bool fail = false;
    if (pk_window_bad(wraw0, wraw1, nflags)) {
        if (threadIdx.x == 0) pk_st(sy + PK_TMO, PK_SITE_WINDOW);
        fail = true;
    }
    bool st_loaded = !halt;
    int k = 0;
    if constexpr (DIST) {
        if (a.init && !halt) {
            const int64_t* slp = pk_launder(a.slice_ptr);
            const int16_t* cop = pk_launder(a.cols);
            const double* vap = pk_launder(a.vals);
            const double* xvp = pk_launder(a.x);
            double gp = 0.0;
#pragma unroll
            for (int j = 0; j < MAXS; ++j) {
                if (j < nreg) {
                    const double q = sell_row_pair<pk_u<MAXS, PROF>(), 0>(s0 + j, lane, slp, cop, vap, xvp, 0, 0, a.uoff, a.ucol);
                    const unsigned row = rb + 64u * j;
                    const bool on = PK_ON(j);
                    double rv = on ? a.b[row] - q : 0.0;
                    const double wj = wl[j * 64];
                    if (cg && wj == 0.0) rv = 0.0;
                    rr[j] = rv;
                    pp[j] = 0.0;
                    ss[j] = 0.0;
                    xl[j * 64] = on ? a.x[row] : 0.0;
                    const double ui = wj * rv;
                    if constexpr (!OD) uo[j] = ui;
                    gp += rv * ui;
                    if (on) {
                        __hip_atomic_store(a.u + row, ui, __ATOMIC_RELAXED, __HIP_MEMORY_SCOPE_AGENT);
                        if (pubmask) pk_publish_row(a, L, pubmask, row, ui);
                    }
                }
                asm volatile("" ::: "memory");
            }
            {
                const double gw = wave_sum(gp);
// ... 92 lines not shown
    (OD ? sell_row_pair_od<pk_u<MAXS, PROF>(), (MODE) == 3 ? 1 : (MODE)>(s0 + (j), lane, slp, cop, vap, uvp, uop, ucp,      \
                                       [&](double acc) { return acc + dg[OD ? (j) : 0] * PK_UO(j); })              \
        : sell_row_pair<pk_u<MAXS, PROF>(), MODE>(s0 + (j), lane, slp, cop, vap, uvp, olo, ohi, uop, ucp))
#define PK_SLOT_DESC(j, jn, more)                                                                                   \
    {                                                                                                               \
        const PkRec nx = pk_rec_load(dsp, s0 + ((more) ? (jn) : (j)));                                              \
        double v;                                                                                                   \
        if (rec.kind() != PKD_LANE)                                                                                 \
            v = sell_row_pair_rec<pk_u_rec<MAXS, PROF>(), 1>(rec, (s0 + (j)) * 64, lane, vap, uvp,                  \
                                                  [&](double acc) { return acc + dg[OD ? (j) : 0] * PK_UO(j); });   \
        else                                                                                                        \
            v = PK_ROW(1, j);                                                                                       \
        if (j < PK_VL) vl[j * 64] = v; else vv[j] = v;                                                              \
        rec = nx;                                                                                                   \
    }
#define PK_SPMV_DESC                                                                               \
    if (!rv) {                                                                                     \
        _Pragma("unroll") for (int j = 0; j < MAXS; ++j) {                                         \
            if (j < nreg) PK_SLOT_DESC(j, j + 1, j + 1 < nreg)                                     \
            asm volatile("" ::: "memory");                                                         \
        }                                                                                          \
    } else {                                                                                       \
        _Pragma("unroll") for (int jj = 0; jj < MAXS; ++jj) {                                      \
            const int j = MAXS - 1 - jj;                                                           \
            if (j < nreg) PK_SLOT_DESC(j, j - 1, j > 0)                                            \
            asm volatile("" ::: "memory");                                                         \
        }                                                                                          \
    }
#define PK_SPMV(MODE)                                                                              \
    if (!rv) {                                                                                     \
        _Pragma("unroll") for (int j = 0; j < MAXS; ++j) {                                         \
            if (j < nreg) {                                                                        \
                const double v = PK_ROW(MODE, j);                                                  \
                if (j < PK_VL) vl[j * 64] = v; else vv[j] = v;                                     \
            }                                                                                      \
            asm volatile("" ::: "memory");                                                         \
        }                                                                                          \
    } else {                                                                                       \
        _Pragma("unroll") for (int jj = 0; jj < MAXS; ++jj) {                                      \
            const int j = MAXS - 1 - jj;                                                           \
            if (j < nreg) {                                                                        \
                const double v = PK_ROW(MODE, j);                                                  \
                if (j < PK_VL) vl[j * 64] = v; else vv[j] = v;                                     \
            }                                                                                      \
            asm volatile("" ::: "memory");                                                         \
        }                                                                                          \
    }
            if constexpr (DESC) {
                PK_SPMV_DESC
            } else if (DIST && ghost) {
                PK_SPMV(3)
            } else {
                PK_SPMV((GSC1 ? 1 : 0))
            }
#undef PK_SPMV
#undef PK_SPMV_DESC
#undef PK_SLOT_DESC
#undef PK_ROW
            if constexpr (PROF) {
                asm volatile("s_waitcnt vmcnt(0) lgkmcnt(0)" ::: "memory");
                wspmv += __builtin_amdgcn_s_memtime() - tw0;
            }
            double dp = 0.0;
#pragma unroll
            for (int j = 0; j < MAXS; ++j) dp += PK_UO(j) * (j < PK_VL ? vl[j * 64] : vv[j]);
            if constexpr (OVF) {
                __builtin_amdgcn_sched_barrier(0);
                for (int q = 0; q < nov; ++q) {
                    const int sq = s0 + MAXS + q;
                    const double v = sell_row_pair<pk_u<MAXS, PROF>(), GSC1>(sq, lane, slp, cop, OD ? a.vals_full : vap, uvp, 0, 0,
                                                                             uop, OD ? a.ucol_full : ucp);
                    const int row = sq * 64 + lane;
                    if (row < nrows) {
                        a.v[row] = v;
                        dp += a.u[row] * v;
                    }
                }
            }
            const int bank = k & 1;
            double* pd = a.part + (size_t)bank * 2 * G;
            PK_MARK(1);
            const double dsum = pk_block_sum(dp, lds16);
            PK_MARK(2);
            if (threadIdx.x == 0) __hip_atomic_store(pd + L, dsum, __ATOMIC_RELAXED, __HIP_MEMORY_SCOPE_AGENT);
            if (!(DIST ? pk_barrier_dist(a, sy, grp, nper, e, &lds_ok, pd, k > 0 ? pd + G : nullptr, G, lds_dg, false)
                       : pk_barrier(sy, grp, nper, e, &lds_ok, pd, k > 0 ? pd + G : nullptr, G, lds_dg, false))) {
                fail = true;
                break;
            }
            elast = e;
            const double d = lds_dg[0];
            if (k > 0) g = lds_dg[1];
            PK_MARK(3);
            double bnew = 0.0;
            bool stop = false;
            if (it > 0) {
                rz_new = g;
                const double nrm = sqrt(g);
                if (L == 0 && threadIdx.x == 0 && a.hist && it - 1 < a.hist_len) a.hist[it - 1] = nrm;
                if (nrm < tol) {
                    status = FEM_PCG_CONVERGED;
                    stop_iter = it;
                    stop = true;
                } else {
                    bnew = cg ? g / (rz + eps) : g / rz;
                    if (cg && (isnan(bnew) || isinf(bnew))) {
                        status = FEM_PCG_BETA_NAN;
                        stop_iter = it;
                        stop = true;
                    }
                }
            }
            if (!stop && it >= max_iter) stop = true;
            double al = 0.0;
            if (!stop) {
                pq = (it == 0) ? d : d - bnew * g / alpha_prev;
                if (cg) {
                    if (fabs(pq) < eps || pq < 0.0) {
                        status = FEM_PCG_BREAKDOWN;
                        stop_iter = it + 1;
                        stop = true;
                    } else {
                        al = g / (pq + eps);
                        if (isnan(al) || isinf(al)) {
                            status = FEM_PCG_ALPHA_NAN;
                            stop_iter = it + 1;
                            stop = true;
                        }
                    }
                } else {
                    al = g / pq;
                }
            }
            if (stop) {
                halt = 1;
                break;
            }
            rz = g;
            alpha_prev = al;
            beta = bnew;
            it += 1;
            PK_MARK(4);
            double gp = 0.0;
            unsigned rbi = rb;
            double* ust = pk_launder(a.u);
            asm volatile("" : "+v"(rbi));
#pragma unroll
            for (int j = 0; j < MAXS; ++j) {
                if (j < nreg) {
                    const double pi = PK_UO(j) + bnew * pp[j];
                    const double si = (j < PK_VL ? vl[j * 64] : vv[j]) + bnew * ss[j];
                    pp[j] = pi;
                    ss[j] = si;
                    xl[j * 64] += al * pi;
                    double ri = rr[j] - al * si;
                    const double wi = wl[j * 64];
                    if (cg && wi == 0.0) ri = 0.0;
                    rr[j] = ri;
                    const double ui = wi * ri;
                    if constexpr (!OD) uo[j] = ui;
                    if (PK_ON(j)) {
                        __hip_atomic_store(ust + (rbi + 64u * j), ui, __ATOMIC_RELAXED, __HIP_MEMORY_SCOPE_AGENT);
                        if constexpr (DIST) {
                            if (pubmask) pk_publish_row(a, L, pubmask, rbi + 64u * j, ui);
                        }
                    }
                    gp += ri * ui;
                }
            }
            if constexpr (OVF) {
                __builtin_amdgcn_sched_barrier(0);
                for (int q = 0; q < nov; ++q) {
                    const int row = (s0 + MAXS + q) * 64 + lane;
                    if (row < nrows) {
                        const double pi = a.u[row] + bnew * a.p[row];
                        const double si = a.v[row] + bnew * a.s[row];
                        a.p[row] = pi;
                        a.s[row] = si;
                        a.x[row] += al * pi;
                        double ri = a.r[row] - al * si;
                        const double wi = a.w[row];
                        if (cg && wi == 0.0) ri = 0.0;
                        a.r[row] = ri;
                        const double ui = wi * ri;
                        __hip_atomic_store(ust + row, ui, __ATOMIC_RELAXED, __HIP_MEMORY_SCOPE_AGENT);
                        gp += ri * ui;
                    }
                }
            }
            {
                const double gw = wave_sum(gp);
                if (lane == 0) lds16[wv] = gw;
            }
            asm volatile("s_waitcnt vmcnt(0)" ::: "memory");
            __syncthreads();
            if (threadIdx.x == 0) {
                double gsum = 0.0;
#pragma unroll
                for (int i = 0; i < PK_WAVES; ++i) gsum += lds16[i];
                __hip_atomic_store(a.part + (size_t)(bank ^ 1) * 2 * G + G + L, gsum, __ATOMIC_RELAXED,
                                   __HIP_MEMORY_SCOPE_AGENT);
                pk_st(uf + Lg * PK_LINE, e);
                if constexpr (DIST) {
                    if (pubmask) {
                        __builtin_amdgcn_fence(__ATOMIC_RELEASE, "");
                        asm volatile("s_waitcnt vmcnt(0)" ::: "memory");
                        pk_publish_flag(a, Lg, pubmask, e);
                    }
                }
            }
            PK_MARK(5);
        }
    }
    auto store_state = [&]() {
        if (!st_loaded) return;
#pragma unroll
        for (int j = 0; j < MAXS; ++j) {
            if (PK_ON(j)) {
                const unsigned row = rb + 64u * j;
                a.r[row] = rr[j];
                a.p[row] = pp[j];
                a.s[row] = ss[j];
                a.x[row] = xl[j * 64];
            }
        }
    };
    if (wv != 0) store_state();
    if (!fail && !halt && k == a.kmax && a.kmax > 0) {
        const unsigned e = ebase + (unsigned)a.kmax + 1;
        const double* pgl = a.part + (size_t)(a.kmax & 1) * 2 * G + G;
        const bool okb = DIST ? pk_barrier_dist(a, sy, grp, nper, e, &lds_ok, pgl, nullptr, G, lds_dg)
                              : pk_barrier(sy, grp, nper, e, &lds_ok, pgl, nullptr, G, lds_dg);
        if (!okb) {
            fail = true;
        } else {
            elast = e;
            g = lds_dg[0];
            if (it > 0) {
                const double nrm = sqrt(g);
                const bool conv = nrm < tol;
                rz_new = g;
                if (conv || it >= max_iter) {
                    if (L == 0 && threadIdx.x == 0 && a.hist && it - 1 < a.hist_len) a.hist[it - 1] = nrm;
                    if (conv) {
                        status = FEM_PCG_CONVERGED;
                        stop_iter = it;
                    }
                    halt = 1;
                }
            }
        }
    }
    if (wv == 0) store_state();
    if constexpr (PROF) {
        asm volatile("s_waitcnt vmcnt(0)" ::: "memory");
        __syncthreads();
        pacc[7] += __builtin_amdgcn_s_memtime() - pt;
        if (threadIdx.x == 0)
            for (int i = 0; i < PK_NPROF; ++i) a.prof[(size_t)L * PK_NPROF + i] = pacc[i];
        if (lane == 0) a.prof[(size_t)G * PK_NPROF + (size_t)L * PK_WAVES + wv] = wspmv;
    }
    if (L == 0 && threadIdx.x == 0) {
        if (fail) {
            stop_iter = (int)pk_ld(sy + PK_TMO);
            status = pk_fail_status((unsigned)stop_iter);
            halt = 1;
        }
        st->iter = it;
        st->halt = halt;
        st->status = status;
        st->stop_iter = stop_iter;
        st->rz = rz;
        st->rz_new = rz_new;
        st->alpha = alpha_prev;
        st->beta = beta;
        st->pq = pq;
        st->red[1] = g;
        st->pk_epoch = elast;
    }
}
#undef PK_ON
#undef PK_MARK
#undef PK_UO

__global__ void k_pk_window_init(int G, int lo_empty, int* __restrict__ win) {
    const int i = blockIdx.x * blockDim.x + threadIdx.x;
    if (i < G) {
        win[i] = lo_empty;
        win[G + i] = -1;
    }
}

__global__ void k_pk_window(int64_t nslices, int64_t nrows, const int64_t* __restrict__ slice_ptr,
                            const int16_t* __restrict__ dcols, int G, int* __restrict__ lo, int* __restrict__ hi) {
    const int64_t W = (int64_t)G * PK_WAVES;
    for (int64_t t = (int64_t)blockIdx.x * blockDim.x + threadIdx.x; t < nslices * 64;
         t += (int64_t)gridDim.x * blockDim.x) {
        const int64_t s = t >> 6;
        const int l = (int)(t & 63);
        const int64_t row = s * 64 + l;
        const int64_t p0 = slice_ptr[s];
        const int w = (int)((slice_ptr[s + 1] - p0) >> 6);
        int dmin = 0, dmax = 0;
        if (row < nrows) {
#pragma unroll 8
            for (int kk = 0; kk < w; ++kk) {
                const int d = dcols[p0 + 64 * kk + l];
                dmin = d < dmin ? d : dmin;
                dmax = d > dmax ? d : dmax;
            }
        }
        int64_t cmin, cmax;
        pk_slice_span(s, nrows, dmin, dmax, &cmin, &cmax);
        auto owner = [&](int64_t r) {
            const int64_t sl = r >> 6;
// ... 53 lines not shown
```

### cuda-powered-mesh-handling-and-iterative-solvers_amd/system.py

```python
from __future__ import annotations

import ctypes
import math
import os
import time
from dataclasses import dataclass

import torch

try:
    from . import _capi as C
except ImportError:
    import _capi as C

I32, I64, F64 = torch.int32, torch.int64, torch.float64


def _scoped(cls):
    import functools

    def wrap(fn):
        @functools.wraps(fn)
        def w(self, *args, **kwargs):
            dev = getattr(self, "device", None)
# ... 1495 lines not shown
            self.set_tuning(tune)

    def _create(self, plain):
        A = self.A
        if getattr(A, "is_matfree", False):
            A.create_context(self.b, self.x, self.w, self._mode, self._tol, self._eps, None, 0,
                             ctypes.c_void_p(self.stream.cuda_stream), self.h)
            self._sl = False
            self.stream.wait_stream(torch.cuda.current_stream(A.device))
            return
        C.check(self.lib.fem_pcg_create(A.g.n_nodes, A.bs, C.ptr(A.g.slice_ptr), C.ptr(A.g.cols),
                                        A.solver_vals_ptr(plain), C.ptr(self.b), C.ptr(self.x), C.ptr(self.w),
                                        self._mode, self._tol, self._eps, None, 0,
                                        ctypes.c_void_p(self.stream.cuda_stream), ctypes.byref(self.h)),
                "fem_pcg_create")
        C.check(self.lib.fem_pcg_set_schedule(self.h, self.schedule), "fem_pcg_set_schedule")
        C.check(self.lib.fem_pcg_set_entries(self.h, A.g.sell_entries), "fem_pcg_set_entries")
        A.attach_cols16(self.h)
        A.attach_layout(self.h, plain)
        self._sl = A.solver_layout and not plain
        if self.constraints is not None:
            C.check(self.lib.fem_pcg_set_constraints(self.h, *self.constraints.args()), "fem_pcg_set_constraints")
        self.stream.wait_stream(torch.cuda.current_stream(A.device))

    def set_tuning(self, flags):
        if self._sl and not (int(flags) & 2):
            self.lib.fem_pcg_destroy(self.h)
            self.h = ctypes.c_void_p()
            self._create(True)
        C.check(self.lib.fem_pcg_set_tuning(self.h, int(flags)), "fem_pcg_set_tuning")

    def finish(self):
        C.check(self.lib.fem_pcg_finish(self.h), "fem_pcg_finish")

    def start(self):
        C.check(self.lib.fem_pcg_start(self.h), "fem_pcg_start")

    def use_graph(self, k):
        C.check(self.lib.fem_pcg_use_graph(self.h, int(k)), "fem_pcg_use_graph")

    def iterate(self, k):
        C.check(self.lib.fem_pcg_iterate(self.h, int(k)), "fem_pcg_iterate")

    def poll(self):
        it, stt, rz = ctypes.c_int(), ctypes.c_int(), ctypes.c_double()
        C.check(self.lib.fem_pcg_poll(self.h, ctypes.byref(it), ctypes.byref(stt), ctypes.byref(rz)), "fem_pcg_poll")
        _check_sync(stt.value)
        return it.value, stt.value, rz.value

    def debug_window(self, L, lo, hi):
        C.check(self.lib.fem_pcg_debug_window(self.h, int(L), int(lo), int(hi)), "fem_pcg_debug_window")

    def effective_schedule(self):
        return int(self.lib.fem_pcg_get_schedule(self.h))

    def uniform_slices(self, s_begin=0, s_end=-1):
        return uniform_slices(self.lib, self.h, s_begin, s_end)

    def offdiag_slices(self):
        c, n, nb = ctypes.c_int64(), ctypes.c_int64(), ctypes.c_int64()
        C.check(self.lib.fem_pcg_offdiag_slices(self.h, ctypes.byref(c), ctypes.byref(n), ctypes.byref(nb)),
                "fem_pcg_offdiag_slices")
        return c.value, n.value, nb.value

    def debug_offdiag_values(self):
        A = self.A
        out = torch.empty(max(A.g.sell_entries, 1), dtype=F64, device=A.device)
        C.check(self.lib.fem_pcg_debug_offdiag(self.h, C.ptr(A.g.rowptr), C.ptr(out)), "fem_pcg_debug_offdiag")
        return out

    def desc_slices(self):
        c, n = ctypes.c_int64(), ctypes.c_int64()
        C.check(self.lib.fem_pcg_desc_slices(self.h, ctypes.byref(c), ctypes.byref(n)), "fem_pcg_desc_slices")
        return c.value, n.value

    def debug_desc_records(self):
        out = torch.empty((max(self.A.g.slice_ptr.numel() - 1, 0), 16), dtype=torch.int32)
        C.check(self.lib.fem_pcg_debug_desc(self.h, ctypes.c_void_p(out.data_ptr())), "fem_pcg_debug_desc")
        return out

    def pipelined(self):
        on = ctypes.c_int()
        C.check(self.lib.fem_pcg_pipelined(self.h, ctypes.byref(on)), "fem_pcg_pipelined")
        return bool(on.value)

    def persist_build(self):
        sl, ov, pk = ctypes.c_int(), ctypes.c_int(), ctypes.c_int()
        C.check(self.lib.fem_pcg_persist_build(self.h, ctypes.byref(sl), ctypes.byref(ov), ctypes.byref(pk)),
                "fem_pcg_persist_build")
        return sl.value, ov.value, pk.value

    def profile(self, k, every=1):
        ms = (ctypes.c_double * 3)()
        n = (ctypes.c_int * 3)()
        C.check(self.lib.fem_pcg_profile(self.h, int(k), int(every), ms, n), "fem_pcg_profile")
        return list(ms), list(n)

    def close(self):
        if self.h:
            self.lib.fem_pcg_destroy(self.h)
            self.h = ctypes.c_void_p()

    def __del__(self):
        try:
            self.close()
        except Exception:
            pass


def newmark_constants(dt, beta=0.25, gamma=0.5, damping=(0.0, 0.0)):
    dt, beta, gamma = float(dt), float(beta), float(gamma)
    if not dt > 0.0:
        raise ValueError(f"Newmark: dt must be > 0, got {dt}")
    if not beta > 0.0 or not gamma >= 0.5:
        raise ValueError(f"Newmark: needs beta > 0 and gamma >= 1/2 (the explicit beta = 0 scheme is out of scope), "
                         f"got beta = {beta}, gamma = {gamma}")
    try:
        alpha, beta_r = (float(d) for d in damping)
    except (TypeError, ValueError):
        raise ValueError(f"Newmark: damping must be the pair (alpha, beta_R), got {damping!r}") from None
    if not alpha >= 0.0 or not beta_r >= 0.0:
        raise ValueError(f"Newmark: the Rayleigh factors must be >= 0, got alpha = {alpha}, beta_R = {beta_r}")
    a0, a1, a2 = 1.0 / (beta * dt * dt), gamma / (beta * dt), 1.0 / (beta * dt)
    a3, a4, a5 = 1.0 / (2.0 * beta) - 1.0, gamma / beta - 1.0, 0.5 * dt * (gamma / beta - 2.0)
    c = dict(dt=dt, beta=beta, gamma=gamma, alpha=alpha, beta_r=beta_r, a0=a0, a1=a1, a2=a2, a3=a3, a4=a4, a5=a5,
             cK=1.0 + a1 * beta_r, cM=a0 + a1 * alpha)
    c["coef"] = [a0, a2, a3, dt * (1.0 - gamma), dt * gamma,
                 a0 + alpha * a1, a2 + alpha * a4, a3 + alpha * a5,
                 beta_r * a1, beta_r * a4, beta_r * a5, dt]
    return c


@dataclass
class TransientResult:
    times: torch.Tensor
    iterations: list
    status: list
    steps_done: int
    rec_u: torch.Tensor = None
    rec_v: torch.Tensor = None
    rec_a: torch.Tensor = None
    energy_steps: list = None
    energies: torch.Tensor = None

    @property
    def converged(self):
        return all(s == C.PCG_CONVERGED for s in self.status)


@_scoped
class NewmarkIntegrator:

    def __init__(self, A: SellMatrix, mass, fixed_mask, dt, beta=0.25, gamma=0.5, damping=(0.0, 0.0), tol=1e-8,
                 rtol=None, max_iter=1000, schedule=None, predictor=False, chunk=32):
        self.c = newmark_constants(dt, beta, gamma, damping)
        self.form, mass = A._mass_form("NewmarkIntegrator", mass)
        if rtol is not None and not float(rtol) > 0.0:
            raise ValueError(f"NewmarkIntegrator: rtol must be > 0, got {rtol}")
        self.lib = C.lib()
        self.A, self.mass, self.device = A, mass, A.device
        self.tol, self.rtol, self.max_iter, self.chunk = float(tol), rtol, int(max_iter), int(chunk)
        self.predictor = bool(predictor)
        self.events = None
        dev, n = A.device, A.n
        self._mv = A._mass_values(self.form, mass)
        self._kv, self._la = A._held_values()
# ... 1199 lines not shown
```

### include/fem355.h

```cpp
#ifndef FEM355_H
#define FEM355_H

#include <stdint.h>

#ifdef __cplusplus
extern "C" {
#endif

typedef void* fem_stream_t;

enum {
    FEM_OK = 0,
    FEM_EBADTYPE = 1,
    FEM_ESINGULAR = 2,
    FEM_EHIP = 3,
    FEM_ERCCL = 4,
    FEM_EARG = 5,
    FEM_ESTATE = 6,
};

enum {
    FEM_PCG_RUNNING = 0,
    FEM_PCG_CONVERGED = 1,
    FEM_PCG_MAXITER = 2,
// ... 147 lines not shown
int fem_vtk_copy(const fem_vtk* v, double* points, int64_t* cells, int64_t* types);
void fem_vtk_free(fem_vtk* v);

int fem_solid_ke(int type, const double* coords, const int64_t* conn, int64_t M, double E, double nu, const double* ip,
                 const double* w, int n_ip, int single, double* Ke, fem_stream_t stream);
int fem_csr_pattern(const int64_t* conn, int64_t M, int npe, int dofs_per_node, int64_t n_nodes, int32_t* rowptr,
                    int32_t* colidx, int32_t* diagpos, int64_t* nnz_out, fem_stream_t stream);
int fem_csr_fill(const double* Ke, const int64_t* conn, int64_t M, int npe, int dpn, int64_t n_nodes,
                 const int32_t* rowptr, const int32_t* colidx, double* vals, fem_stream_t stream);
int fem_spmv_csr(const int32_t* rowptr, const int32_t* colidx, const double* vals, const double* x, double* y,
                 int64_t n, fem_stream_t stream);
int fem_pcg_csr(const int32_t* rowptr, const int32_t* colidx, const double* vals, int64_t n, const double* b,
                double* x, const double* dinv, const uint8_t* fixed_mask, double tol, int max_iter, double eps,
                int mode, int* iters_out, int* status_out, double* res_hist_out, fem_stream_t stream);

int fem_spmv(int64_t nrows, int bs, const int64_t* slice_ptr, const int32_t* cols, const double* vals,
             const double* x, double* y, fem_stream_t stream);
int fem_sell_delta16(const int32_t* cols, int64_t nrows, const int64_t* slice_ptr, int16_t* dcols, int32_t* overflow,
                     fem_stream_t stream);
int fem_spmv16(int64_t nrows, int bs, const int64_t* slice_ptr, const int16_t* dcols, const double* vals,
               const double* x, double* y, fem_stream_t stream);
int fem_stream_copy(const double* src, double* dst, int64_t n, int grid, fem_stream_t stream);
int fem_stream_read(const double* src, double* out, int64_t n, int grid, fem_stream_t stream);

typedef struct fem_pcg fem_pcg;
int fem_pcg_create(int64_t nrows, int bs, const int64_t* slice_ptr, const int32_t* cols, const double* vals,
                   const double* b, double* x, const double* w, int mode, double tol, double eps,
                   double* hist, int64_t hist_len, fem_stream_t stream, fem_pcg** out);
int fem_pcg_start(fem_pcg* s);
int fem_pcg_iterate(fem_pcg* s, int k);
int fem_pcg_poll(fem_pcg* s, int* iters, int* status, double* rz);
int fem_pcg_debug_window(fem_pcg* s, int L, int lo, int hi);
int fem_pcg_sync_site(fem_pcg* s, int* site);
int fem_pcg_scalars(fem_pcg* s, double* out6);
int fem_pcg_solve(fem_pcg* s, int max_iter, int chunk, int* iters, int* status, double* rz);
int fem_pcg_set_schedule(fem_pcg* s, int sched);
int fem_pcg_set_entries(fem_pcg* s, int64_t entries);
int fem_pcg_set_tol(fem_pcg* s, double tol);
int fem_pcg_get_schedule(fem_pcg* s);
int fem_pcg_uniform_slices(fem_pcg* s, int64_t s_begin, int64_t s_end, int64_t* uniform, int64_t* nslices,
                           int64_t* index_bytes);
int fem_pcg_offdiag_slices(fem_pcg* s, int64_t* od_slices, int64_t* nslices, int64_t* bytes);
int fem_pcg_debug_offdiag(fem_pcg* s, const int32_t* rowptr, double* vals);
int fem_pcg_desc_slices(fem_pcg* s, int64_t* desc_slices, int64_t* nslices);
int fem_pcg_debug_desc(fem_pcg* s, uint32_t* records);
int fem_sell_sl_pattern(int64_t nrows, const int64_t* slice_ptr, const int16_t* dcols, int G, int16_t* pcols,
                        int16_t* ucol, int32_t* uoff, int32_t* win, fem_stream_t stream);
int fem_assemble_tet4_sl(const double* coords, const int64_t* conn, double E, double nu, int bs,
                         const int32_t* inc_ptr, const int32_t* inc, int64_t N, const int32_t* rowptr,
                         const int32_t* colidx, const int64_t* slice_ptr, const int32_t* uoff, const int16_t* ucol,
                         int store, int max_width, double* svals, int64_t* bad_idx, fem_stream_t stream);
int fem_assemble_tet4_scaled(const double* coords, const int64_t* conn, double E, double nu, int bs,
                             const int32_t* inc_ptr, const int32_t* inc, int64_t N, const int32_t* rowptr,
                             const int32_t* colidx, const int64_t* csr2sell, const int64_t* slice_ptr, int store,
                             int max_width, const double* scale, double* vals, int64_t* bad_idx,
                             fem_stream_t stream);
int fem_assemble_tet4_scaled_sl(const double* coords, const int64_t* conn, double E, double nu, int bs,
                                const int32_t* inc_ptr, const int32_t* inc, int64_t N, const int32_t* rowptr,
                                const int32_t* colidx, const int64_t* slice_ptr, const int32_t* uoff,
                                const int16_t* ucol, int store, int max_width, const double* scale, double* svals,
                                int64_t* bad_idx, fem_stream_t stream);
int fem_assemble_from_ke_sl(const double* Ke, const int64_t* conn, int npe, const int32_t* inc_ptr, const int32_t* inc,
                            int64_t N, const int32_t* rowptr, const int32_t* colidx, const int64_t* slice_ptr,
                            int store, int max_width, double* svals, fem_stream_t stream);
int fem_assemble_from_ke_sym(const double* Kp, const int64_t* conn, int npe, const int32_t* inc_ptr,
                             const int32_t* inc, int64_t N, const int32_t* rowptr, const int32_t* colidx,
                             const int64_t* slice_ptr, int store, int max_width, int layout_a, double* vals,
                             fem_stream_t stream);
int fem_assemble_from_ke_mass_sl(const double* Ke, const double* Me, const int64_t* conn, int npe,
                                 const int32_t* inc_ptr, const int32_t* inc, int64_t N, const int32_t* rowptr,
                                 const int32_t* colidx, const int64_t* slice_ptr, int store, int max_width,
                                 double* svals, double* mvals, fem_stream_t stream);
int fem_jacobi_sl(const double* svals, int bs, const int32_t* rowptr, const int32_t* diagpos,
                  const int64_t* slice_ptr, const int32_t* uoff, const int16_t* ucol, int64_t nrows,
                  const uint8_t* mask, double* w, fem_stream_t stream);
int fem_spmv_sl(int64_t nrows, int bs, const int64_t* slice_ptr, const int16_t* pcols, const double* svals,
                const int32_t* uoff, const int16_t* ucol, const double* x, double* y, fem_stream_t stream);
int fem_sell_sl_unpair(int64_t nrows, int bs, const int64_t* slice_ptr, const int16_t* dcols, const int32_t* uoff,
                       const int16_t* ucol, const int32_t* rowptr, const double* svals, double* vals,
                       fem_stream_t stream);
int fem_pcg_set_layout(fem_pcg* s, const double* svals, const int16_t* pcols, const int32_t* uoff,
                       const int16_t* ucol, const int32_t* win, int G);
int fem_pcg_persist_build(fem_pcg* s, int* slots, int* overflow, int* pack);
int fem_pcg_pipelined(fem_pcg* s, int* on);
int fem_pcg_persist_profile(fem_pcg* s, int k, unsigned long long* host_out, int* grid);
int fem_pcg_set_constraints(fem_pcg* s, int order, int64_t R, const int64_t* rbe2_slave, const int64_t* rbe2_master,
                            int64_t S, const int64_t* spc_dof, const double* spc_val, int64_t G,
                            const int64_t* r3_ptr, const int64_t* r3_master, const double* r3_wsum,
                            const int64_t* r3_slave, const double* r3_w);
int fem_enforce_constraints(double* x, double* r, int64_t n, int order, int64_t R, const int64_t* rbe2_slave,
                            const int64_t* rbe2_master, int64_t S, const int64_t* spc_dof, const double* spc_val,
                            int64_t G, const int64_t* r3_ptr, const int64_t* r3_master, const double* r3_wsum,
                            const int64_t* r3_slave, const double* r3_w, fem_stream_t stream);
enum { FEM_TUNE_REVERSE = 1, FEM_TUNE_PAIR = 2, FEM_TUNE_PK_SC1 = 4, FEM_TUNE_PK_PACK = 8, FEM_TUNE_C1F = 16,
       FEM_TUNE_PK_COOP = 32, FEM_TUNE_DIST_FINE = 64, FEM_TUNE_PK_UNI = 128, FEM_TUNE_PK_WIDE = 256,
       FEM_TUNE_DIST_DROP = 512, FEM_TUNE_UPD1 = 1024, FEM_TUNE_U2_HOLD = 2048, FEM_TUNE_U2_SMALL = 4096,
       FEM_TUNE_MF_GATHER = 8192, FEM_TUNE_PK_GV = 16384, FEM_TUNE_PK_OFFDIAG = 32768,
       FEM_TUNE_PK_DESC = 65536 };
int fem_pcg_set_tuning(fem_pcg* s, int flags);
int fem_pcg_set_cols16(fem_pcg* s, const int16_t* dcols);
int fem_pcg_finish(fem_pcg* s);
int fem_pcg_use_graph(fem_pcg* s, int k);
int fem_pcg_profile(fem_pcg* s, int k, int every, double* ms, int* n);
void fem_pcg_destroy(fem_pcg* s);
int fem_pcg_set_rows(fem_pcg* s, int nranks, int rank, const int64_t* slice_split, int grid);
int fem_pcg_comm_block(fem_pcg* s, void** base, int64_t* bytes);
int fem_pcg_col_window(fem_pcg* s, int64_t* lo, int64_t* hi);
int fem_pcg_set_peers(fem_pcg* s, void* const* bases, const int64_t* need_lo, const int64_t* need_hi);
int fem_pcg_dist_debug(fem_pcg* s, int which, int32_t* host_out, int64_t n);
int fem_stream_create_cu(int part, int nparts, void** stream);
int fem_stream_destroy(void* stream);
int fem_pcg_set_prof(fem_pcg* s, unsigned long long* dev_buf);
int fem_ipc_handle(void* ptr, char* out64);
int fem_ipc_open(const char* h64, void** ptr);
int fem_ipc_close(void* ptr);
int fem_pcg_release_cache(void);
int fem_release_scratch(void);

int fem_comm_unique_id(char* out128);
int fem_comm_init(int nranks, int rank, const char* id128, void** comm);
int fem_comm_destroy(void* comm);
int fem_allreduce_sum(void* comm, double* buf, int64_t n, fem_stream_t stream);
int fem_halo_pack(const double* v, int bs, const int32_t* imap, int64_t nI, double* buf, fem_stream_t stream);
int fem_halo_unpack(double* v, int bs, const int32_t* ipos, int64_t nrows, const double* buf, fem_stream_t stream);
int fem_halo_sum(void* comm, double* v, int bs, const int32_t* imap, int64_t nI, const int32_t* ipos, int64_t nrows,
                 double* buf, fem_stream_t stream);
int fem_pcg_set_dist(fem_pcg* s, int enable, void* comm, int64_t nI, const int32_t* imap, const int32_t* ipos,
                     const uint8_t* own);
int fem_pcg_set_dist_variant(fem_pcg* s, int variant);
int fem_pcg_set_p2p(fem_pcg* s, int nranks, int npeer, const int* peer_rank, const int64_t* peer_cnt,
                    const int32_t* csrc, const int32_t* ssrc);
int fem_pcg_p2p_buffers(fem_pcg* s, double** psend, double** precv, int64_t* total);
int fem_p2p_deliver(fem_pcg* const* ctx, int P, fem_stream_t stream);
int fem_pcg_dist_phase(fem_pcg* s, int phase);
int fem_pcg_dist_buffer(fem_pcg* s, int phase, double** ptr, int64_t* n);
int fem_group_allreduce(double* const* dev_ptr_array, int P, int64_t n, fem_stream_t stream);

typedef struct fem_mf fem_mf;
int fem_mf_create(const double* coords, const int64_t* conn, int64_t M, int64_t N, int kind, double E, double nu,
                  int64_t* bad_idx, fem_stream_t stream, fem_mf** out);
int fem_mf_destroy(fem_mf* m);
int fem_mf_apply(fem_mf* m, const double* x, double* y, fem_stream_t stream);
int fem_mf_diag(fem_mf* m, double* d, fem_stream_t stream);
int fem_mf_info(fem_mf* m, int64_t* out6);
int fem_mf_order(fem_mf* m, int32_t* eorder, int32_t* cptr, int32_t* sbase, int32_t* cnode, fem_stream_t stream);
int fem_pcg_set_operator_mf(fem_pcg* s, fem_mf* m);

int fem_spmm(int64_t nrows, int bs, int nv, const int64_t* slice_ptr, const int32_t* cols, const int16_t* dcols,
             const double* vals, const double* X, double* Y, fem_stream_t stream);
typedef struct fem_mpcg fem_mpcg;
int fem_mpcg_create(int64_t nrows, int bs, int nv, int nactive, const int64_t* slice_ptr, const int32_t* cols,
                    const int16_t* dcols, const double* vals, const double* B, double* X, const double* w, int mode,
                    const double* tol, double eps, double* hist, int64_t hist_len, fem_stream_t stream,
                    fem_mpcg** out);
int fem_mpcg_solve(fem_mpcg* s, int max_iter, int chunk, int* iters, int* status, double* rz);
int fem_mpcg_scalars(fem_mpcg* s, double* out);
void fem_mpcg_destroy(fem_mpcg* s);

#define FEM_COARSE_MAX_AGG 512
int fem_coarse_restrict(int64_t nrows, int bs, int k, const int32_t* agg_ptr, const int32_t* agg_nodes,
                        const double* rel, const double* w, const double* r, double* c, fem_stream_t stream);
int fem_coarse_apply(int64_t nrows, int bs, int k, const int32_t* agg, const double* rel, const double* w,
                     const double* Einv, const double* c, const double* r, double* y, double* z, fem_stream_t stream);
int fem_coarse_galerkin_count(int64_t nrows, int bs, const int64_t* slice_ptr, const int32_t* cols,
                              const int16_t* dcols, const int32_t* agg, int64_t* count, fem_stream_t stream);
int fem_coarse_galerkin(int64_t nrows, int bs, int k, const int64_t* slice_ptr, const int32_t* cols,
                        const int16_t* dcols, const double* vals, const int32_t* agg, const double* rel,
                        const double* w, const int64_t* offset, int64_t* keys, double* rec, fem_stream_t stream);
int fem_coarse_galerkin_sum(int64_t nkeys, int k, const int64_t* ukeys, const int64_t* key_ptr, const int64_t* order,
                            const double* rec, double* E, fem_stream_t stream);
typedef struct fem_pcg2 fem_pcg2;
int fem_pcg2_create(int64_t nrows, int bs, const int64_t* slice_ptr, const int32_t* cols, const int16_t* dcols,
                    const double* vals, const double* b, double* x, const double* w, int k, const int32_t* agg,
                    const int32_t* agg_ptr, const int32_t* agg_nodes, const double* rel, const double* Einv, double tol,
                    double* hist, int64_t hist_len, fem_stream_t stream, fem_pcg2** out);
int fem_pcg2_solve(fem_pcg2* s, int max_iter, int chunk, int* iters, int* status, double* rz);
int fem_pcg2_scalars(fem_pcg2* s, double* out6);
void fem_pcg2_destroy(fem_pcg2* s);

int fem_refine_edge_slots(const int64_t* conn, int64_t M, const int64_t* uedges, int64_t E, int32_t* eid,
                          int64_t* minslot, fem_stream_t stream);
// ... 142 lines not shown
```

Before: 25440 CG iterations/s.

## Replace persistent-PCG grid barrier with epoch-tagged granule reductions

Adds a granule reduction path to the single-GPU persistent PCG kernel. Each block publishes its partial dot product as two 64-bit words tagged with the epoch. Reducer waves poll those words with 16-byte buffer loads until every tag matches, so the atomic counter barrier and the separate partial-sum read are no longer needed. It is enabled by default for 1-slot and max-slot builds. The cost is more polling traffic on the granule array and another set of kernel instantiations, and the sync state is reset when the reduction kind switches.

Result: faster. 26490 CG iterations/s (median of 6 runs) (+4.1%).

```diff
diff --git a/cuda-powered-mesh-handling-and-iterative-solvers_amd/_capi.py b/cuda-powered-mesh-handling-and-iterative-solvers_amd/_capi.py
--- a/cuda-powered-mesh-handling-and-iterative-solvers_amd/_capi.py
+++ b/cuda-powered-mesh-handling-and-iterative-solvers_amd/_capi.py
@@ -22,7 +22,9 @@
 TUNE_PK_GV = 16384
 TUNE_PK_OFFDIAG = 32768
 TUNE_PK_DESC = 65536
-TUNE_DEFAULT = 1 | 2 | 4 | 8 | 128 | TUNE_UPD1 | TUNE_PK_OFFDIAG | TUNE_PK_DESC
+TUNE_PK_GRAN = 131072
+TUNE_PK_GRAN_SMALL = 262144
+TUNE_DEFAULT = 1 | 2 | 4 | 8 | 128 | TUNE_UPD1 | TUNE_PK_OFFDIAG | TUNE_PK_DESC | TUNE_PK_GRAN
 KIND_ELASTIC, KIND_POISSON, KIND_MASS = 0, 1, 2
 ISO_SUM, ISO_STACK, ISO_VOLUME, ISO_MASS = 0, 1, 2, 3
 MASS_SELL, MASS_DIAG = 0, 1
@@ -135,6 +137,7 @@
     "fem_pcg_desc_slices": (_I, [_P, _P, _P]),
     "fem_pcg_debug_desc": (_I, [_P, _P]),
     "fem_pcg_persist_build": (_I, [_P, ctypes.POINTER(_I), ctypes.POINTER(_I), ctypes.POINTER(_I)]),
+    "fem_pcg_persist_granules": (_I, [_P, ctypes.POINTER(_I)]),
     "fem_pcg_pipelined": (_I, [_P, ctypes.POINTER(_I)]),
     "fem_sell_sl_pattern": (_I, [_L, _P, _P, _I, _P, _P, _P, _P, _P]),
     "fem_assemble_tet4_sl": (_I, [_P, _P, _D, _D, _I, _P, _P, _L, _P, _P, _P, _P, _P, _I, _I, _P, _P, _P]),
diff --git a/cuda-powered-mesh-handling-and-iterative-solvers_amd/csrc/pcg.hip b/cuda-powered-mesh-handling-and-iterative-solvers_amd/csrc/pcg.hip
--- a/cuda-powered-mesh-handling-and-iterative-solvers_amd/csrc/pcg.hip
+++ b/cuda-powered-mesh-handling-and-iterative-solvers_amd/csrc/pcg.hip
@@ -1736,6 +1736,8 @@
     int32_t* pk_win;
     double* pk_part;
     unsigned* pk_sync;
+    pk_u64* pk_gran;
+    int pk_red_kind;
     int pk_ovf;
     double* pk_v;
     int pk_od;
@@ -2587,12 +2589,14 @@
     const void* fn;
     size_t lds;
     bool desc;
+    bool gran;
 };
 
-template <int MAXS, bool PROF, bool GSC1, bool OVF = false, bool DIST = false, bool OD = false, bool DESC = false>
+template <int MAXS, bool PROF, bool GSC1, bool OVF = false, bool DIST = false, bool OD = false, bool DESC = false,
+          bool GRAN = false>
 static PkBuild pk1_build() {
     return {DIST ? PKF_BS1_DIST : PKF_BS1, MAXS, PROF, GSC1, OVF, DIST, OD,
-            (const void*)k_pcg_persist<MAXS, PROF, GSC1, OVF, DIST, OD, DESC>, PK_LDS, DESC};
+            (const void*)k_pcg_persist<MAXS, PROF, GSC1, OVF, DIST, OD, DESC, GRAN>, PK_LDS, DESC, GRAN};
 }
 template <bool OVF, bool DIST>
 static PkBuild pk3_build() {
@@ -2629,6 +2633,12 @@
     pk1_build<4, false, true, false, false, true, true>(),
     pk1_build<PK_MAXS, false, true, false, false, true, true>(),
     pk1_build<PK_MAXS, true, true, false, false, true, true>(),
+    pk1_build<1, false, true, false, false, true, true, true>(),
+    pk1_build<2, false, true, false, false, true, true, true>(),
+    pk1_build<4, false, true, false, false, true, true, true>(),
+    pk1_build<PK_MAXS, false, true, false, false, true, true, true>(),
+    pk1_build<PK_MAXS, true, true, false, false, true, true, true>(),
+    pk1_build<PK_MAXS, false, true, true, false, true, false, true>(),
     pk1_build<1, false, true, false, true>(),
     pk1_build<2, false, true, false, true>(),
     pk1_build<PK_MAXS_DIST, false, true, false, true>(),
@@ -2645,10 +2655,10 @@
 };
 
 static const PkBuild* pk_find(PkFamily fam, int slots, bool prof, bool gsc1, bool ovf, bool dist, bool od,
-                              bool desc = false) {
+                              bool desc = false, bool gran = false) {
     for (const PkBuild& b : PK_BUILDS)
         if (b.fam == fam && b.slots == slots && b.prof == prof && b.gsc1 == gsc1 && b.ovf == ovf && b.dist == dist &&
-            b.od == od && b.desc == desc)
+            b.od == od && b.desc == desc && b.gran == gran)
             return &b;
     return nullptr;
 }
@@ -2689,6 +2699,8 @@
     const bool small = pack >= 1 && pack <= 4 && !(s->tune & FEM_TUNE_PK_WIDE) && !prof && !ovf && gsc1;
     const int slots = !small ? PK_MAXS : pack == 1 ? 1 : pack == 2 ? 2 : 4;
     const bool desc = s->pk_od && s->pk_desc_on && gsc1 && !ovf;
+    if ((s->tune & FEM_TUNE_PK_GRAN) && (slots == 1 || slots == PK_MAXS || (s->tune & FEM_TUNE_PK_GRAN_SMALL)))
+        if (const PkBuild* b = pk_find(PKF_BS1, slots, prof, gsc1, ovf, false, s->pk_od != 0, desc, true)) return {b, pack};
     return {pk_find(PKF_BS1, slots, prof, gsc1, ovf, false, s->pk_od != 0, desc), pack};
 }
 static PkPlan persist_plan(const fem_pcg* s, bool prof) { return persist_plan(s, prof, s->pk_gv && s->bs == 1); }
@@ -2931,7 +2943,7 @@
     }
     fem_pcg* s = new fem_pcg();
     s->tune = FEM_TUNE_REVERSE | FEM_TUNE_PAIR | FEM_TUNE_PK_SC1 | FEM_TUNE_PK_PACK | FEM_TUNE_PK_UNI | FEM_TUNE_UPD1 |
-              FEM_TUNE_PK_OFFDIAG | FEM_TUNE_PK_DESC;
+              FEM_TUNE_PK_OFFDIAG | FEM_TUNE_PK_DESC | FEM_TUNE_PK_GRAN;
     s->nrows = nrows;
     s->bs = bs;
     s->nslices = cdiv(nrows, 64);
@@ -3341,12 +3353,15 @@
         pool_free(s->pk_win, s->stream);
         pool_free(s->pk_part, s->stream);
         pool_free(s->pk_sync, s->stream);
+        pool_free(s->pk_gran, s->stream);
         s->pk_win = nullptr;
         s->pk_part = nullptr;
         s->pk_sync = nullptr;
+        s->pk_gran = nullptr;
         FEM_HIP(pool_alloc((void**)&s->pk_win, sizeof(int32_t) * 2 * G, s->stream, s->bs == 1));
         FEM_HIP(pool_alloc((void**)&s->pk_part, sizeof(double) * 4 * G, s->stream, s->bs == 1));
         FEM_HIP(pool_alloc((void**)&s->pk_sync, sizeof(unsigned) * pk_sync_words(G), s->stream, s->bs == 1));
+        FEM_HIP(pool_alloc((void**)&s->pk_gran, sizeof(pk_u64) * pk_gran_words(G), s->stream, s->bs == 1));
         s->pk_grid = G;
         s->pk_win_ok = 0;
     }
@@ -3425,8 +3440,10 @@
 
 static int persist_reset_sync(fem_pcg* s) {
     FEM_HIP(hipMemsetAsync(s->pk_sync, 0, sizeof(unsigned) * pk_sync_words(s->pk_grid), s->stream));
+    FEM_HIP(hipMemsetAsync(s->pk_gran, 0, sizeof(pk_u64) * pk_gran_words(s->pk_grid), s->stream));
     FEM_HIP(hipMemsetAsync(&s->st->pk_epoch, 0, sizeof(unsigned), s->stream));
     s->pk_epochs = 0;
+    s->pk_red_kind = 0;
     return FEM_OK;
 }
 
@@ -3473,6 +3490,7 @@
     a.vals_full = s->pvals;
     a.ucol_full = uni ? s->pucol : nullptr;
     a.desc = plan.b->desc ? s->pk_desc : nullptr;
+    a.gran = plan.b->gran ? s->pk_gran : nullptr;
     return a;
 }
 
@@ -3514,6 +3532,13 @@
         set_error("persistent PCG: no build for this context (%d slices per wave)", plan.pack);
         return FEM_ESTATE;
     }
+    const int red_kind = plan.b->gran ? 2 : 1;
+    if (!s->pd && s->pk_red_kind && s->pk_red_kind != red_kind) {
+        const int rc = persist_reset_sync(s);
+        if (rc) return rc;
+        s->pk_epochs = k + 1;
+    }
+    s->pk_red_kind = red_kind;
     PkArgs a = pk_args(s, plan, k, prof);
     s->pd_init_pending = 0;
     GvArgs g;
@@ -3534,6 +3559,14 @@
 
 int fem_pcg_pipelined(fem_pcg* s, int* on) {
     *on = (s && s->persist && s->pk_gv) ? 1 : 0;
+    return FEM_OK;
+}
+
+int fem_pcg_persist_granules(fem_pcg* s, int* on) {
+    *on = 0;
+    if (!s || !s->persist || s->pk_grid <= 0) return FEM_OK;
+    const PkPlan plan = persist_plan(s, false);
+    *on = (plan.b && plan.b->gran) ? 1 : 0;
     return FEM_OK;
 }
 
@@ -3686,6 +3719,7 @@
             return FEM_EARG;
         }
         FEM_HIP(hipMemsetAsync(s->pk_sync, 0, sizeof(unsigned) * pk_sync_words(s->pk_grid), s->stream));
+        FEM_HIP(hipMemsetAsync(s->pk_gran, 0, sizeof(pk_u64) * pk_gran_words(s->pk_grid), s->stream));
         FEM_HIP(hipMemsetAsync(s->pd_block, 0, (size_t)s->pd_block_bytes, s->stream));
         FEM_HIP(hipMemsetAsync(&s->st->pk_epoch, 0, sizeof(unsigned), s->stream));
         s->pk_epochs = 0;
@@ -4207,9 +4241,12 @@
     pool_free(s->pk_win, s->stream);
     pool_free(s->pk_part, s->stream);
     pool_free(s->pk_sync, s->stream);
+    pool_free(s->pk_gran, s->stream);
     FEM_HIP(pool_alloc((void**)&s->pk_win, sizeof(int32_t) * (2 * G + 2), s->stream, true));
     FEM_HIP(pool_alloc((void**)&s->pk_part, sizeof(double) * 4 * G, s->stream, true));
     FEM_HIP(pool_alloc((void**)&s->pk_sync, sizeof(unsigned) * pk_sync_words(G), s->stream, true));
+    FEM_HIP(pool_alloc((void**)&s->pk_gran, sizeof(pk_u64) * pk_gran_words(G), s->stream, true));
+    FEM_HIP(hipMemsetAsync(s->pk_gran, 0, sizeof(pk_u64) * pk_gran_words(G), s->stream));
     s->pk_grid = G;
     std::vector<int32_t> lohi(2 * (size_t)G + 2);
     for (int i = 0; i < G; ++i) {
@@ -4420,6 +4457,7 @@
     pool_free(s->pk_win, s->stream);
     pool_free(s->pk_part, s->stream);
     pool_free(s->pk_sync, s->stream);
+    pool_free(s->pk_gran, s->stream);
     pool_free(s->pk_v, s->stream);
     pool_free(s->pk_ovals, s->stream);
     pool_free(s->pk_oucol, s->stream);
diff --git a/cuda-powered-mesh-handling-and-iterative-solvers_amd/csrc/pcg_persist.hpp b/cuda-powered-mesh-handling-and-iterative-solvers_amd/csrc/pcg_persist.hpp
--- a/cuda-powered-mesh-handling-and-iterative-solvers_amd/csrc/pcg_persist.hpp
+++ b/cuda-powered-mesh-handling-and-iterative-solvers_amd/csrc/pcg_persist.hpp
@@ -1,119 +1,7 @@
 #pragma once
-#include "sell_pair.hpp"
+#include "pcg_persist_sync.hpp"
 
 namespace fem {
-
-constexpr int PK_MAXS = 7;
-constexpr int PK_U = 2;
-template <int MAXS, bool PROF>
-constexpr int pk_u() { return MAXS <= 1 ? 8 : (MAXS <= 4 && !PROF) ? 4 : PK_U; }
-template <int MAXS, bool PROF>
-constexpr int pk_u_rec() { return MAXS <= 1 ? 4 : pk_u<MAXS, PROF>(); }
-constexpr int PK_LINE = 32;
-enum { PK_GRP = 0, PK_TOP = 8 * PK_LINE, PK_GEN = 9 * PK_LINE, PK_TMO = 17 * PK_LINE, PK_UFLAG = 18 * PK_LINE };
-constexpr uint64_t PK_WAIT_TICKS = 200000000ull;
-constexpr uint64_t PK_RANK_WAIT_TICKS = 500000000ull;
-__device__ __forceinline__ uint64_t pk_now() { return __builtin_amdgcn_s_memrealtime(); }
-__device__ __forceinline__ bool pk_expired(uint64_t t0, uint64_t ticks) { return pk_now() - t0 > ticks; }
-constexpr int PK_NPROF = 8;
-constexpr size_t PK_LDS_HEAD = 256;
-constexpr int PK_VL = 5;
-constexpr size_t PK_LDS = PK_LDS_HEAD + sizeof(double) * (2 * PK_MAXS + PK_VL) * PK_WAVES * 64;
-static_assert(PK_LDS <= 160 * 1024, "persistent PCG: LDS over the 160 KB of a CU");
-
-template <class T>
-__device__ __forceinline__ T* pk_launder(T* p) {
-    __attribute__((address_space(1))) T* q = (__attribute__((address_space(1))) T*)p;
-    asm volatile("" : "+s"(q));
-    return (T*)q;
-}
-
-__device__ __forceinline__ unsigned pk_ld(const unsigned* p) {
-    return __hip_atomic_load(p, __ATOMIC_RELAXED, __HIP_MEMORY_SCOPE_AGENT);
-}
-__device__ __forceinline__ void pk_st(unsigned* p, unsigned v) {
-    __hip_atomic_store(p, v, __ATOMIC_RELAXED, __HIP_MEMORY_SCOPE_AGENT);
-}
-
-__device__ __forceinline__ bool pk_wait_ge(const unsigned* p, unsigned target, unsigned* tmo) {
-    const uint64_t t0 = pk_now();
-    for (unsigned spins = 0;; ++spins) {
-        if (pk_ld(p) >= target) return true;
-        if ((spins & 63) == 63 && pk_ld(tmo)) return false;
-        if ((spins & 63) == 63 && pk_expired(t0, PK_WAIT_TICKS)) {
-            pk_st(tmo, 1u + 16u * (target / NXCD));
-            return false;
-        }
-        __builtin_amdgcn_s_sleep(2);
-    }
-}
-
-__device__ __forceinline__ double pk_sum(const double* part, int n) {
-    const int lane = threadIdx.x & 63;
-    double v = 0.0;
-    for (int i = lane; i < n; i += 64) v += __hip_atomic_load(part + i, __ATOMIC_RELAXED, __HIP_MEMORY_SCOPE_AGENT);
-    return wave_sum(v);
-}
-
-__device__ __forceinline__ bool pk_barrier(unsigned* sy, int grp, unsigned nper, unsigned e, int* lds_ok,
-                                           const double* pd, const double* pg, int G, double* out,
-                                           bool entry_sync = true) {
-    if (entry_sync) __syncthreads();
-    if (threadIdx.x < 64) {
-        int okv = 0;
-        if (threadIdx.x == 0) {
-            asm volatile("s_waitcnt vmcnt(0)" ::: "memory");
-            unsigned* tmo = sy + PK_TMO;
-            bool ok;
-            const unsigned old = __hip_atomic_fetch_add(sy + PK_GRP + grp * PK_LINE, 1u, __ATOMIC_RELAXED,
-                                                        __HIP_MEMORY_SCOPE_AGENT);
-            if (old == e * nper - 1)
-                for (int r = 0; r < NXCD; ++r)
-                    __hip_atomic_fetch_add(sy + PK_GEN + r * PK_LINE, 1u, __ATOMIC_RELAXED, __HIP_MEMORY_SCOPE_AGENT);
-            ok = pk_wait_ge(sy + PK_GEN + grp * PK_LINE, e * NXCD, tmo);
-            okv = ok ? 1 : 0;
-        }
-        okv = __builtin_amdgcn_readfirstlane(okv);
-        if (okv && pd) {
-            const int lane = threadIdx.x & 63;
-            double vd = 0.0, vg = 0.0;
-            if (pg) {
-#pragma unroll 4
-                for (int i = lane; i < G; i += 64) {
-                    const double a = __hip_atomic_load(pd + i, __ATOMIC_RELAXED, __HIP_MEMORY_SCOPE_AGENT);
-                    const double b = __hip_atomic_load(pg + i, __ATOMIC_RELAXED, __HIP_MEMORY_SCOPE_AGENT);
-                    vd += a;
-                    vg += b;
-                }
-            } else {
-#pragma unroll 4
-                for (int i = lane; i < G; i += 64) vd += __hip_atomic_load(pd + i, __ATOMIC_RELAXED, __HIP_MEMORY_SCOPE_AGENT);
-            }
-            const double d = wave_sum(vd);
-            const double g = pg ? wave_sum(vg) : 0.0;
-            if (threadIdx.x == 0) {
-                out[0] = d;
-                out[1] = g;
-            }
-        }
-        if (threadIdx.x == 0) *lds_ok = okv;
-    }
-    __syncthreads();
-    return *lds_ok != 0;
-}
-
-__device__ __forceinline__ double pk_block_sum(double v, double* lds16) {
-    v = wave_sum(v);
-    const int w = threadIdx.x >> 6;
-    if ((threadIdx.x & 63) == 0) lds16[w] = v;
-    __syncthreads();
-    double t = 0.0;
-    if (threadIdx.x == 0) {
-#pragma unroll
-        for (int i = 0; i < PK_WAVES; ++i) t += lds16[i];
-    }
-    return t;
-}
 
 constexpr int PK_MAX_RANKS = 8;
 
@@ -152,6 +40,7 @@
     const double* vals_full;
     const int16_t* ucol_full;
     const PkDesc* desc;
+    pk_u64* gran;
 };
 
 __device__ __forceinline__ double pk_mul_rn(double a, double b) {
@@ -256,8 +145,10 @@
 
 #define PK_ON(j) ((j) < nreg && lane < nrows - (s0 + (j)) * 64)
 
-template <int MAXS, bool PROF, bool GSC1, bool OVF = false, bool DIST = false, bool OD = false, bool DESC = false>
+template <int MAXS, bool PROF, bool GSC1, bool OVF = false, bool DIST = false, bool OD = false, bool DESC = false,
+          bool GRAN = false>
 __global__ void __launch_bounds__(PK_T) k_pcg_persist(PkArgs a) {
+    static_assert(!(GRAN && DIST), "granule reduction: single-GPU builds (the DIST barrier carries the rank exchange)");
     static_assert(!DIST || (GSC1 && !OVF), "distributed persistent PCG: sc1 gathers, no overflow build");
     static_assert(!(DIST && OD), "distributed persistent PCG: no diagonal-free stream");
     static_assert(!DESC || (OD && GSC1 && !OVF), "descriptor records: the diagonal-free sc1 builds without overflow");
@@ -275,6 +166,7 @@
     double* lds16 = pk_lds_raw;
     int& lds_ok = *reinterpret_cast<int*>(pk_lds_raw + PK_WAVES);
     double* lds_dg = pk_lds_raw + PK_WAVES + 2;
+    static_assert(PKG_OK2 * sizeof(int) == 32, "granule build: the second verdict word sits at byte 160 of the head");
     double* pk_lds = pk_lds_raw + PK_LDS_HEAD / sizeof(double);
     const int G = gridDim.x;
     const unsigned nper = (unsigned)(G / NXCD);
@@ -304,6 +196,7 @@
     double* wl = pk_lds + PK_WAVES * MAXS * 64 + wv * MAXS * 64 + lane;
     double* vl = pk_lds + 2 * PK_WAVES * MAXS * 64 + wv * PK_VL * 64 + lane;
     unsigned* sy = a.sync;
+    pk_u64* const gran = GRAN ? a.gran : nullptr;
     PcgState* st = a.st;
     unsigned* uf = DIST ? reinterpret_cast<unsigned*>(a.peer[a.rank] + a.off_flag) : sy + PK_UFLAG;
     const int Lg = DIST ? a.rank * G + L : L;
@@ -562,9 +455,16 @@
             PK_MARK(1);
             const double dsum = pk_block_sum(dp, lds16);
             PK_MARK(2);
-            if (threadIdx.x == 0) __hip_atomic_store(pd + L, dsum, __ATOMIC_RELAXED, __HIP_MEMORY_SCOPE_AGENT);
-            if (!(DIST ? pk_barrier_dist(a, sy, grp, nper, e, &lds_ok, pd, k > 0 ? pd + G : nullptr, G, lds_dg, false)
-                       : pk_barrier(sy, grp, nper, e, &lds_ok, pd, k > 0 ? pd + G : nullptr, G, lds_dg, false))) {
+            bool okb;
+            if (GRAN) {
+                if (threadIdx.x == 0) pk_gran_put(pk_gran_at(gran, G, L, e, 0), e, dsum);
+                okb = pk_gran_reduce(gran, sy, e, &lds_ok, G, k > 0 ? PKG_DG : PKG_D, lds_dg, false);
+            } else {
+                if (threadIdx.x == 0) __hip_atomic_store(pd + L, dsum, __ATOMIC_RELAXED, __HIP_MEMORY_SCOPE_AGENT);
+                okb = DIST ? pk_barrier_dist(a, sy, grp, nper, e, &lds_ok, pd, k > 0 ? pd + G : nullptr, G, lds_dg, false)
+                           : pk_barrier(sy, grp, nper, e, &lds_ok, pd, k > 0 ? pd + G : nullptr, G, lds_dg, false);
+            }
+            if (!okb) {
                 fail = true;
                 break;
             }
@@ -678,8 +578,11 @@
                 double gsum = 0.0;
 #pragma unroll
                 for (int i = 0; i < PK_WAVES; ++i) gsum += lds16[i];
-                __hip_atomic_store(a.part + (size_t)(bank ^ 1) * 2 * G + G + L, gsum, __ATOMIC_RELAXED,
-                                   __HIP_MEMORY_SCOPE_AGENT);
+                if (GRAN)
+                    pk_gran_put(pk_gran_at(gran, G, L, e + 1, 2), e + 1, gsum);
+                else
+                    __hip_atomic_store(a.part + (size_t)(bank ^ 1) * 2 * G + G + L, gsum, __ATOMIC_RELAXED,
+                                       __HIP_MEMORY_SCOPE_AGENT);
                 pk_st(uf + Lg * PK_LINE, e);
                 if constexpr (DIST) {
                     if (pubmask) {
@@ -709,8 +612,9 @@
     if (!fail && !halt && k == a.kmax && a.kmax > 0) {
         const unsigned e = ebase + (unsigned)a.kmax + 1;
         const double* pgl = a.part + (size_t)(a.kmax & 1) * 2 * G + G;
-        const bool okb = DIST ? pk_barrier_dist(a, sy, grp, nper, e, &lds_ok, pgl, nullptr, G, lds_dg)
-                              : pk_barrier(sy, grp, nper, e, &lds_ok, pgl, nullptr, G, lds_dg);
+        const bool okb = GRAN   ? pk_gran_reduce(gran, sy, e, &lds_ok, G, PKG_G, lds_dg)
+                         : DIST ? pk_barrier_dist(a, sy, grp, nper, e, &lds_ok, pgl, nullptr, G, lds_dg)
+                                : pk_barrier(sy, grp, nper, e, &lds_ok, pgl, nullptr, G, lds_dg);
         if (!okb) {
             fail = true;
         } else {
diff --git a/cuda-powered-mesh-handling-and-iterative-solvers_amd/csrc/pcg_persist_sync.hpp b/cuda-powered-mesh-handling-and-iterative-solvers_amd/csrc/pcg_persist_sync.hpp
--- /dev/null
+++ b/cuda-powered-mesh-handling-and-iterative-solvers_amd/csrc/pcg_persist_sync.hpp
@@ -0,0 +1,228 @@
+#pragma once
+#include "sell_pair.hpp"
+
+namespace fem {
+
+constexpr int PK_MAXS = 7;
+constexpr int PK_U = 2;
+template <int MAXS, bool PROF>
+constexpr int pk_u() { return MAXS <= 1 ? 8 : (MAXS <= 4 && !PROF) ? 4 : PK_U; }
+template <int MAXS, bool PROF>
+constexpr int pk_u_rec() { return MAXS <= 1 ? 4 : pk_u<MAXS, PROF>(); }
+constexpr int PK_LINE = 32;
+enum { PK_GRP = 0, PK_TOP = 8 * PK_LINE, PK_GEN = 9 * PK_LINE, PK_TMO = 17 * PK_LINE, PK_UFLAG = 18 * PK_LINE };
+constexpr uint64_t PK_WAIT_TICKS = 200000000ull;
+constexpr uint64_t PK_RANK_WAIT_TICKS = 500000000ull;
+__device__ __forceinline__ uint64_t pk_now() { return __builtin_amdgcn_s_memrealtime(); }
+__device__ __forceinline__ bool pk_expired(uint64_t t0, uint64_t ticks) { return pk_now() - t0 > ticks; }
+constexpr int PK_NPROF = 8;
+constexpr size_t PK_LDS_HEAD = 256;
+constexpr int PK_VL = 5;
+constexpr size_t PK_LDS = PK_LDS_HEAD + sizeof(double) * (2 * PK_MAXS + PK_VL) * PK_WAVES * 64;
+static_assert(PK_LDS <= 160 * 1024, "persistent PCG: LDS over the 160 KB of a CU");
+
+template <class T>
+__device__ __forceinline__ T* pk_launder(T* p) {
+    __attribute__((address_space(1))) T* q = (__attribute__((address_space(1))) T*)p;
+    asm volatile("" : "+s"(q));
+    return (T*)q;
+}
+
+__device__ __forceinline__ unsigned pk_ld(const unsigned* p) {
+    return __hip_atomic_load(p, __ATOMIC_RELAXED, __HIP_MEMORY_SCOPE_AGENT);
+}
+__device__ __forceinline__ void pk_st(unsigned* p, unsigned v) {
+    __hip_atomic_store(p, v, __ATOMIC_RELAXED, __HIP_MEMORY_SCOPE_AGENT);
+}
+
+__device__ __forceinline__ bool pk_wait_ge(const unsigned* p, unsigned target, unsigned* tmo) {
+    const uint64_t t0 = pk_now();
+    for (unsigned spins = 0;; ++spins) {
+        if (pk_ld(p) >= target) return true;
+        if ((spins & 63) == 63 && pk_ld(tmo)) return false;
+        if ((spins & 63) == 63 && pk_expired(t0, PK_WAIT_TICKS)) {
+            pk_st(tmo, 1u + 16u * (target / NXCD));
+            return false;
+        }
+        __builtin_amdgcn_s_sleep(2);
+    }
+}
+
+__device__ __forceinline__ double pk_sum(const double* part, int n) {
+    const int lane = threadIdx.x & 63;
+    double v = 0.0;
+    for (int i = lane; i < n; i += 64) v += __hip_atomic_load(part + i, __ATOMIC_RELAXED, __HIP_MEMORY_SCOPE_AGENT);
+    return wave_sum(v);
+}
+
+__device__ __forceinline__ bool pk_barrier(unsigned* sy, int grp, unsigned nper, unsigned e, int* lds_ok,
+                                           const double* pd, const double* pg, int G, double* out,
+                                           bool entry_sync = true) {
+    if (entry_sync) __syncthreads();
+    if (threadIdx.x < 64) {
+        int okv = 0;
+        if (threadIdx.x == 0) {
+            asm volatile("s_waitcnt vmcnt(0)" ::: "memory");
+            unsigned* tmo = sy + PK_TMO;
+            bool ok;
+            const unsigned old = __hip_atomic_fetch_add(sy + PK_GRP + grp * PK_LINE, 1u, __ATOMIC_RELAXED,
+                                                        __HIP_MEMORY_SCOPE_AGENT);
+            if (old == e * nper - 1)
+                for (int r = 0; r < NXCD; ++r)
+                    __hip_atomic_fetch_add(sy + PK_GEN + r * PK_LINE, 1u, __ATOMIC_RELAXED, __HIP_MEMORY_SCOPE_AGENT);
+            ok = pk_wait_ge(sy + PK_GEN + grp * PK_LINE, e * NXCD, tmo);
+            okv = ok ? 1 : 0;
+        }
+        okv = __builtin_amdgcn_readfirstlane(okv);
+        if (okv && pd) {
+            const int lane = threadIdx.x & 63;
+            double vd = 0.0, vg = 0.0;
+            if (pg) {
+#pragma unroll 4
+                for (int i = lane; i < G; i += 64) {
+                    const double a = __hip_atomic_load(pd + i, __ATOMIC_RELAXED, __HIP_MEMORY_SCOPE_AGENT);
+                    const double b = __hip_atomic_load(pg + i, __ATOMIC_RELAXED, __HIP_MEMORY_SCOPE_AGENT);
+                    vd += a;
+                    vg += b;
+                }
+            } else {
+#pragma unroll 4
+                for (int i = lane; i < G; i += 64) vd += __hip_atomic_load(pd + i, __ATOMIC_RELAXED, __HIP_MEMORY_SCOPE_AGENT);
+            }
+            const double d = wave_sum(vd);
+            const double g = pg ? wave_sum(vg) : 0.0;
+            if (threadIdx.x == 0) {
+                out[0] = d;
+                out[1] = g;
+            }
+        }
+        if (threadIdx.x == 0) *lds_ok = okv;
+    }
+    __syncthreads();
+    return *lds_ok != 0;
+}
+
+__device__ __forceinline__ double pk_block_sum(double v, double* lds16) {
+    v = wave_sum(v);
+    const int w = threadIdx.x >> 6;
+    if ((threadIdx.x & 63) == 0) lds16[w] = v;
+    __syncthreads();
+    double t = 0.0;
+    if (threadIdx.x == 0) {
+#pragma unroll
+        for (int i = 0; i < PK_WAVES; ++i) t += lds16[i];
+    }
+    return t;
+}
+
+typedef unsigned long long pk_u64;
+constexpr unsigned PK_SITE_GRAN = 5u;
+constexpr int PK_GRAN_STRIDE = 4;
+constexpr bool PK_GRAN_L16 = true;
+constexpr int PK_GRAN_NEAR = 8;
+#define PK_GRAN_NAP 8
+constexpr size_t pk_gran_words(int G, int stride = PK_GRAN_STRIDE) { return (size_t)2 * G * stride; }
+
+__device__ __forceinline__ void pk_gran_put(pk_u64* g, unsigned e, double v) {
+    const pk_u64 b = (pk_u64)__double_as_longlong(v), t = (pk_u64)e << 32;
+    __hip_atomic_store(g, t | (b & 0xffffffffull), __ATOMIC_RELAXED, __HIP_MEMORY_SCOPE_AGENT);
+    __hip_atomic_store(g + 1, t | (b >> 32), __ATOMIC_RELAXED, __HIP_MEMORY_SCOPE_AGENT);
+}
+__device__ __forceinline__ double pk_gran_val(pk_u64 lo, pk_u64 hi) {
+    return __longlong_as_double((long long)((lo & 0xffffffffull) | (hi << 32)));
+}
+template <bool L16>
+__device__ __forceinline__ void pk_gran_ld(const pk_u64* bank, size_t bytes, unsigned i, pk_u64& lo, pk_u64& hi) {
+    if constexpr (L16) {
+        typedef unsigned pk_v4u __attribute__((ext_vector_type(4)));
+        const __amdgpu_buffer_rsrc_t rs = __builtin_amdgcn_make_buffer_rsrc((void*)bank, 0, (int)bytes, 0x00027000);
+        const pk_v4u r = __builtin_amdgcn_raw_buffer_load_b128(rs, (int)(i * sizeof(pk_u64)), 0, (int)0x80000010u);
+        lo = (pk_u64)r.x | ((pk_u64)r.y << 32);
+        hi = (pk_u64)r.z | ((pk_u64)r.w << 32);
+    } else {
+        lo = __hip_atomic_load(bank + i, __ATOMIC_RELAXED, __HIP_MEMORY_SCOPE_AGENT);
+        hi = __hip_atomic_load(bank + i + 1, __ATOMIC_RELAXED, __HIP_MEMORY_SCOPE_AGENT);
+    }
+}
+
+template <int STRIDE, bool L16, bool MASKED, bool COUNT = false>
+__device__ __forceinline__ bool pk_gran_sum(const pk_u64* bank, int G, unsigned e, int woff, unsigned* tmo, double* sum,
+                                            unsigned long long* moved = nullptr) {
+    const int lane = threadIdx.x & 63;
+    const pk_u64 tag = e;
+    const size_t bytes = (size_t)G * STRIDE * sizeof(pk_u64);
+    double v = 0.0;
+    bool ok = true;
+    for (int base = 0; base < G && ok; base += 256) {
+        pk_u64 w[4][2] = {};
+        bool miss[4];
+#pragma unroll
+        for (int r = 0; r < 4; ++r) miss[r] = base + lane + 64 * r < G;
+        const uint64_t t0 = pk_now();
+        for (unsigned spins = 0;; ++spins) {
+            asm volatile("" ::: "memory");
+#pragma unroll
+            for (int r = 0; r < 4; ++r) {
+                if (miss[r]) {
+                    pk_gran_ld<L16>(bank, bytes, (unsigned)((base + lane + 64 * r) * STRIDE + woff), w[r][0], w[r][1]);
+                    if constexpr (COUNT) *moved += 16;
+                }
+            }
+            bool any = false;
+#pragma unroll
+            for (int r = 0; r < 4; ++r) {
+                if (miss[r]) {
+                    const bool m = (w[r][0] >> 32) == tag && (w[r][1] >> 32) == tag;
+                    if (MASKED) miss[r] = !m;
+                    any = any || !m;
+                }
+            }
+            const int nmiss = __popcll(__ballot(any));
+            if (nmiss == 0) break;
+            if ((spins & 63) == 63) {
+                if (__builtin_amdgcn_readfirstlane(pk_ld(tmo))) ok = false;
+                else if (pk_expired(t0, PK_WAIT_TICKS)) {
+                    if (lane == 0) pk_st(tmo, PK_SITE_GRAN + 16u * e);
+                    ok = false;
+                }
+                if (!ok) break;
+            }
+            if (nmiss > PK_GRAN_NEAR) __builtin_amdgcn_s_sleep(PK_GRAN_NAP);
+            else __builtin_amdgcn_s_sleep(1);
+        }
+#pragma unroll
+        for (int r = 0; r < 4; ++r)
+            if (ok && base + lane + 64 * r < G) v += pk_gran_val(w[r][0], w[r][1]);
+    }
+    *sum = wave_sum(v);
+    return ok;
+}
+
+__device__ __forceinline__ bool pk_gran_collect(const pk_u64* gran, unsigned* sy, unsigned e, int G, int woff,
+                                                double* sum) {
+    return pk_gran_sum<PK_GRAN_STRIDE, PK_GRAN_L16, true>(gran + (size_t)(e & 1u) * G * PK_GRAN_STRIDE, G, e, woff,
+                                                          sy + PK_TMO, sum);
+}
+enum { PKG_D = 0, PKG_DG = 1, PKG_G = 2 };
+constexpr int PKG_OK2 = 8;
+__device__ __forceinline__ bool pk_gran_reduce(const pk_u64* gran, unsigned* sy, unsigned e, int* ok, int G, int what,
+                                               double* out, bool entry_sync = true) {
+    if (entry_sync) __syncthreads();
+    const int wvx = __builtin_amdgcn_readfirstlane(threadIdx.x >> 6);
+    const bool second = what == PKG_DG && wvx == PK_WAVES - 1;
+    if (wvx == 0 || second) {
+        double sum;
+        const bool okw = pk_gran_collect(gran, sy, e, G, (second || what == PKG_G) ? 2 : 0, &sum);
+        if ((threadIdx.x & 63) == 0) {
+            if (okw) out[second ? 1 : 0] = sum;
+            ok[second ? PKG_OK2 : 0] = okw ? 1 : 0;
+        }
+    }
+    __syncthreads();
+    return ok[0] != 0 && (what != PKG_DG || ok[PKG_OK2] != 0);
+}
+__device__ __forceinline__ pk_u64* pk_gran_at(pk_u64* gran, int G, int L, unsigned e, int woff) {
+    return gran + ((size_t)(e & 1u) * G + L) * PK_GRAN_STRIDE + woff;
+}
+
+}
diff --git a/cuda-powered-mesh-handling-and-iterative-solvers_amd/system.py b/cuda-powered-mesh-handling-and-iterative-solvers_amd/system.py
--- a/cuda-powered-mesh-handling-and-iterative-solvers_amd/system.py
+++ b/cuda-powered-mesh-handling-and-iterative-solvers_amd/system.py
@@ -1601,6 +1601,11 @@
     def pipelined(self):
         on = ctypes.c_int()
         C.check(self.lib.fem_pcg_pipelined(self.h, ctypes.byref(on)), "fem_pcg_pipelined")
+        return bool(on.value)
+
+    def persist_granules(self):
+        on = ctypes.c_int()
+        C.check(self.lib.fem_pcg_persist_granules(self.h, ctypes.byref(on)), "fem_pcg_persist_granules")
         return bool(on.value)
 
     def persist_build(self):
diff --git a/include/fem355.h b/include/fem355.h
--- a/include/fem355.h
+++ b/include/fem355.h
@@ -253,6 +253,7 @@
 int fem_pcg_set_layout(fem_pcg* s, const double* svals, const int16_t* pcols, const int32_t* uoff,
                        const int16_t* ucol, const int32_t* win, int G);
 int fem_pcg_persist_build(fem_pcg* s, int* slots, int* overflow, int* pack);
+int fem_pcg_persist_granules(fem_pcg* s, int* on);
 int fem_pcg_pipelined(fem_pcg* s, int* on);
 int fem_pcg_persist_profile(fem_pcg* s, int k, unsigned long long* host_out, int* grid);
 int fem_pcg_set_constraints(fem_pcg* s, int order, int64_t R, const int64_t* rbe2_slave, const int64_t* rbe2_master,
@@ -267,7 +268,7 @@
        FEM_TUNE_PK_COOP = 32, FEM_TUNE_DIST_FINE = 64, FEM_TUNE_PK_UNI = 128, FEM_TUNE_PK_WIDE = 256,
        FEM_TUNE_DIST_DROP = 512, FEM_TUNE_UPD1 = 1024, FEM_TUNE_U2_HOLD = 2048, FEM_TUNE_U2_SMALL = 4096,
        FEM_TUNE_MF_GATHER = 8192, FEM_TUNE_PK_GV = 16384, FEM_TUNE_PK_OFFDIAG = 32768,
-       FEM_TUNE_PK_DESC = 65536 };
+       FEM_TUNE_PK_DESC = 65536, FEM_TUNE_PK_GRAN = 131072, FEM_TUNE_PK_GRAN_SMALL = 262144 };
 int fem_pcg_set_tuning(fem_pcg* s, int flags);
 int fem_pcg_set_cols16(fem_pcg* s, const int16_t* dcols);
 int fem_pcg_finish(fem_pcg* s);
```
